# huggingface/diffusers

Measured on AMD Instinct MI355X. Metric: images/sec @ SDXL-base 1024x1024 50-step EulerDiscrete CFG bf16, higher is better.
Workload: dtype bf16; 1 GPU; SDXL-base-1.0 U-Net (2567 M params) x 50 EulerDiscrete steps, CFG 5.0 (batch 2), 128x128 latents + AutoencoderKL decode to 1024x1024; 1 prompt per GPU; global_batch=1, parallelism=dp1 (independent prompts, replicas), denoise_steps=50, output_type=pt, hip_graph=True, output_finite=True, rccl_ranks=1, tuned_live=0, cpu_binding=none

## Files before the change

### diffusers_amd/csrc/gemm.hip

```cpp
#include "gemm_kernel.cuh"
#include "gemm2_shared.cuh"

namespace da_gemm {
int dispatch_conv(const da_gemm_params& p, int tile, int staging, hipStream_t s);
}
namespace da_gemm2 {
int dispatch_lin(const da_gemm_params& p, int tile, int staging, hipStream_t s);
int dispatch_conv(const da_gemm_params& p, int tile, int staging, hipStream_t s);
}
namespace da_gemm3 {
int dispatch_lin(const da_gemm_params& p, int tile, int staging, hipStream_t s);
}

namespace {

struct TileShape {
  int bm, bn, waves;
};
constexpr TileShape kTiles[] = {{0, 0, 0},      {128, 128, 4}, {64, 128, 4},  {128, 64, 4}, {64, 64, 4},
                                {256, 128, 8},  {128, 256, 8}, {256, 256, 8}, {128, 128, 8},
                                {128, 128, 8},  {128, 80, 8},  {128, 160, 8}, {80, 128, 8}, {128, 64, 8},
                                {128, 320, 8},  {256, 128, 8}, {128, 256, 8}, {256, 160, 8}, {256, 256, 8}, {256, 320, 8},
                                {256, 256, 8},  {256, 320, 8}};
static_assert(sizeof(kTiles) / sizeof(kTiles[0]) == DA_TILE_COUNT, "kTiles / DA_TILE_* mismatch");
inline bool is_k3(int tile) { return tile == DA_TILE_K3_256x256 || tile == DA_TILE_K3_256x320; }
inline bool is_k2(int tile) { return tile >= DA_TILE_K2_128x128 && !is_k3(tile); }
constexpr int kNumTiles = sizeof(kTiles) / sizeof(kTiles[0]);

int pick_tile(const da_gemm_params& p) {
  auto nblk = [&](int t) {
    return (long)((p.M + kTiles[t].bm - 1) / kTiles[t].bm) * ((p.N + kTiles[t].bn - 1) / kTiles[t].bn);
  };
  const bool geglu = (p.act == DA_ACT_GEGLU || p.act == DA_ACT_GEGLU_TANH);
  const bool narrow = !geglu && ((p.N & 127) != 0) && ((p.N % 128) <= 64);
  if (narrow) return (nblk(DA_TILE_128x64) >= 200) ? DA_TILE_128x64 : DA_TILE_64x64;
  if (nblk(DA_TILE_256x128) >= 480) return DA_TILE_256x128;
  if (nblk(DA_TILE_128x128) >= 128) return DA_TILE_128x128;
  if (nblk(DA_TILE_64x128) >= 128 || geglu) return DA_TILE_64x128;
  return DA_TILE_64x64;
}

int validate_conv(const da_gemm_params& p) {
  if (p.C1 <= 0 || (p.C1 & 63) || (p.C2 & 63) || p.C2 < 0) return DA_ERR_UNSUPPORTED;
  if (p.conv != 1 && p.conv != 3) return DA_ERR_UNSUPPORTED;
  if (p.K != p.conv * p.conv * (p.C1 + p.C2)) return DA_ERR_INVALID;
  if (p.stride != 1 && p.stride != 2) return DA_ERR_UNSUPPORTED;
  if (p.up != 0 && p.up != 1) return DA_ERR_INVALID;
  if (p.Hin <= 0 || p.Win <= 0 || p.Hout <= 0 || p.Wout <= 0) return DA_ERR_INVALID;
  if (p.M % (p.Hout * p.Wout)) return DA_ERR_INVALID;
  return DA_OK;
}

int validate(da_gemm_params& p) {
  if (p.M <= 0 || p.N <= 0 || p.K <= 0) return DA_ERR_INVALID;
  if ((p.K & 63) || (p.N & 3) || (p.ldc & 3)) return DA_ERR_UNSUPPORTED;
  if (!p.A || !p.W || !p.C) return DA_ERR_INVALID;
  if (p.residual && (p.ldr & 3)) return DA_ERR_UNSUPPORTED;
  if (p.rowvec && (p.rows_per_batch <= 0 || (p.ld_rowvec & 3))) return DA_ERR_INVALID;
  if (p.gate && (p.rows_per_batch <= 0 || (p.ld_gate & 3))) return DA_ERR_INVALID;
  if (p.alpha == 0.0f) p.alpha = 1.0f;
  if (p.out_scale == 0.0f) p.out_scale = 1.0f;
  if (p.conv) {
    const int v = validate_conv(p);
    if (v != DA_OK) return v;
    if (p.C2 > 0 && !p.A2) return DA_ERR_INVALID;
  } else {
    if ((p.lda & 7) || (p.ldw & 7)) return DA_ERR_UNSUPPORTED;
  }
  if ((p.act == DA_ACT_GEGLU || p.act == DA_ACT_GEGLU_TANH) &&
      ((p.N & 127) || p.out_f32 || p.residual || p.rowvec || p.gate || p.bias_rows))
    return DA_ERR_UNSUPPORTED;
  if (p.act < 0 || p.act > DA_ACT_GEGLU_TANH) return DA_ERR_INVALID;
  if (p.split_k < 0 || p.split_k > DA_SPLITK_MAX) return DA_ERR_INVALID;
  if (p.split_k > 1 && (p.stats_out || p.ln_stats)) return DA_ERR_UNSUPPORTED;
  if (p.k_valid < 0 || (p.k_valid > 0 && (p.k_valid > (p.conv ? p.C1 : p.K) || (p.conv && p.C2 != 0)))) return DA_ERR_INVALID;
  if (p.stats_out && (p.conv || p.out_f32 || p.act == DA_ACT_GEGLU || p.act == DA_ACT_GEGLU_TANH || p.stats_ld <= 0 || (p.stats_ld & 1)))
    return DA_ERR_UNSUPPORTED;
  if (p.ln_stats && (p.conv || !p.ln_s || !p.ln_c || p.ln_parts <= 0 || p.ln_parts > 4 * DA_LN_PAIR_LOADS ||
                     p.ln_stats_ld < 2 * DA_LN_MAX_PARTS || (p.ln_stats_ld & 3)))
    return DA_ERR_INVALID;
  return DA_OK;
}

int stats_parts(const da_gemm_params& p, int tile) {
  if (is_k2(tile)) {
    const int band = (tile == DA_TILE_K2_128x80 || tile == DA_TILE_K2_128x160) ? 80 : 0;
    return band ? (p.N + band - 1) / band : 0;
  }
  return (p.N + kTiles[tile].bn - 1) / kTiles[tile].bn;
}

bool tile_ok(const da_gemm_params& p, int tile) {
  if (tile <= 0 || tile >= kNumTiles) return false;
  if (is_k3(tile)) {
    if (p.conv || p.split_k > 1 || p.stats_out || (p.ln_stats && tile != DA_TILE_K3_256x320) || p.vt || p.xa_k) return false;
    if (tile == DA_TILE_K3_256x320)
      return (p.act == DA_ACT_GEGLU || p.act == DA_ACT_GEGLU_TANH) && (p.M % 256) == 0 && (p.N % 320) == 0 && !(p.ldc & 7) &&
             !((size_t)p.C & 15);
    return true;
  }
  if (is_k2(tile)) {
    const bool geglu = (p.act == DA_ACT_GEGLU || p.act == DA_ACT_GEGLU_TANH);
    const bool geglu_ok = tile == DA_TILE_K2_128x128 || tile == DA_TILE_K1_256x128 || tile == DA_TILE_K1_128x256 ||
                          tile == DA_TILE_K1_256x256 || tile == DA_TILE_K1_256x320 || (tile == DA_TILE_K1_128x320 && !p.conv);
    const bool lnf_lin = tile == DA_TILE_K2_128x80 || tile == DA_TILE_K2_128x160;
    const bool lnf_cons = lnf_lin || tile == DA_TILE_K1_128x256 || tile == DA_TILE_K1_256x128;
    if (p.xa_k) return !p.conv && p.split_k <= 1 && !geglu && !p.stats_out && !p.vt && tile == DA_TILE_K2_128x128;
    if (p.vt) return !p.conv && p.split_k <= 1 && !geglu && !p.stats_out && lnf_cons;
    if (p.stats_out || p.ln_stats) {
      if (p.conv || p.split_k > 1) return false;
      if (p.stats_out && (geglu || !lnf_lin)) return false;
      return geglu ? tile == DA_TILE_K1_128x320 : lnf_cons;
    }
    return p.split_k <= 1 && (!geglu || geglu_ok) &&
           !(p.conv && (tile == DA_TILE_K2_80x128 || tile == DA_TILE_K1_256x256 || tile == DA_TILE_K1_256x320));
  }
  if (p.vt || p.xa_k) return false;
  if ((p.act == DA_ACT_GEGLU || p.act == DA_ACT_GEGLU_TANH) &&
      (tile == DA_TILE_128x64 || tile == DA_TILE_64x64 || tile == DA_TILE_128x128_W8))
    return false;
  if (tile == DA_TILE_256x256 && (p.stats_out || p.ln_stats)) return false;
  return true;
}

__global__ __launch_bounds__(256) void touch_kernel(const uint4* __restrict__ src, size_t n, unsigned* __restrict__ sink) {
  unsigned acc = 0;
  for (size_t i = (size_t)blockIdx.x * 256 + threadIdx.x; i < n; i += (size_t)gridDim.x * 256) {
    const uint4 v = src[i];
    acc ^= v.x ^ v.y ^ v.z ^ v.w;
  }
  if (acc == 0x9e3779b9u) sink[0] = acc;
}

int run(const da_gemm_params& p, int tile, int staging, hipStream_t s, const da_gemm_params* pb = nullptr) {
  if (is_k3(tile)) return pb ? DA_ERR_UNSUPPORTED : da_gemm3::dispatch_lin(p, tile, staging, s);
  if (is_k2(tile)) {
    if (pb) return DA_ERR_UNSUPPORTED;
    return p.conv ? da_gemm2::dispatch_conv(p, tile, staging, s) : da_gemm2::dispatch_lin(p, tile, staging, s);
  }
  if (p.conv) return pb ? DA_ERR_UNSUPPORTED : da_gemm::dispatch_conv(p, tile, staging, s);
  return da_gemm::dispatch<false>(p, tile, staging, s, pb);
}

}

extern "C" int da_gemm_bf16(const da_gemm_params* pp, void* stream) {
  if (!pp) return DA_ERR_INVALID;
  da_gemm_params p = *pp;
  const int v = validate(p);
  if (v != DA_OK) return v;
  int tile = p.tile;
  if (tile == DA_TILE_AUTO) tile = pick_tile(p);
  if (!tile_ok(p, tile)) return DA_ERR_UNSUPPORTED;
  if (p.stats_out && (stats_parts(p, tile) <= 0 || p.stats_ld < 2 * stats_parts(p, tile))) return DA_ERR_INVALID;
  return run(p, tile, p.staging, (hipStream_t)stream);
}

extern "C" int da_gemm_stats_parts(const da_gemm_params* pp) {
  if (!pp || pp->N <= 0) return 0;
  int tile = pp->tile;
  if (tile == DA_TILE_AUTO) tile = pick_tile(*pp);
  if (tile <= 0 || tile >= kNumTiles) return 0;
  return stats_parts(*pp, tile);
}

extern "C" int da_conv_chunk_channels(const da_gemm_params* pp, int tile) {
  if (!pp || !pp->conv || pp->M <= 0 || pp->N <= 0) return -DA_ERR_INVALID;
  const da_gemm_params& p = *pp;
  const int v = validate_conv(p);
  if (v != DA_OK) return -v;
  if (!is_k2(tile) || !tile_ok(p, tile)) return -DA_ERR_UNSUPPORTED;
  return da_gemm2::conv_chunk_channels(p, kTiles[tile].bm, kTiles[tile].bn);
}

extern "C" int da_gemm_pair_bf16(const da_gemm_params* pa, const da_gemm_params* pb, void* stream) {
  if (!pa || !pb) return DA_ERR_INVALID;
  da_gemm_params a = *pa, b = *pb;
  int v = validate(a);
  if (v != DA_OK) return v;
  v = validate(b);
  if (v != DA_OK) return v;
  if (a.conv || b.conv || a.split_k > 1 || b.split_k > 1) return DA_ERR_UNSUPPORTED;
  int tile = a.tile;
  if (tile == DA_TILE_AUTO) tile = pick_tile(a);
  if (!tile_ok(a, tile) || !tile_ok(b, tile)) return DA_ERR_UNSUPPORTED;
  return run(a, tile, a.staging, (hipStream_t)stream, &b);
}

extern "C" int da_gemm_tune(const da_gemm_params* pp, const da_gemm_params* pair, void* stream, int iters, void* scratch,
                            size_t scratch_bytes, int* best_tile, int* best_staging, int* best_split, float* best_us) {
  if (!pp || !best_tile || !best_staging) return DA_ERR_INVALID;
  da_gemm_params p = *pp;
  int v = validate(p);
  if (v != DA_OK) return v;
  da_gemm_params pb{};
  if (pair) {
    pb = *pair;
    v = validate(pb);
    if (v != DA_OK) return v;
    if (p.conv || pb.conv) return DA_ERR_UNSUPPORTED;
  }
  if (iters <= 0) iters = 3;
  hipStream_t s = (hipStream_t)stream;
  hipEvent_t e0, e1;
  if (hipEventCreate(&e0) != hipSuccess || hipEventCreate(&e1) != hipSuccess) return DA_ERR_LAUNCH;
  float best = 3.0e38f;
  int bt = 0, bs = 0, bk = 1;
  static const int stagings[] = {DA_STAGE_LDS_DIRECT, DA_STAGE_LDS_DIRECT3, DA_STAGE_LDS_DIRECT4, DA_STAGE_LDS_DIRECT6,
                                 DA_STAGE_LDS_DIRECT8, DA_STAGE_PINGPONG, DA_STAGE_PINGPONG3};
  constexpr int n_stagings = sizeof(stagings) / sizeof(stagings[0]);
  static const int splits[] = {1, 2, 3, 4, 6, 8, 12, 16, 24};
  const int n_splits = (best_split && !pair && p.workspace && p.sync_flags) ? (int)(sizeof(splits) / sizeof(splits[0])) : 1;
  const int family = pp->tile;
  for (int spi = 0; spi < n_splits; ++spi) {
    const int split = splits[spi];
    p.split_k = split;
    for (int tile = 1; tile < kNumTiles; ++tile) {
      if ((family == DA_TILE_FAMILY_1 && (is_k2(tile) || is_k3(tile))) || (family == DA_TILE_FAMILY_K2 && !is_k2(tile) && !is_k3(tile))) continue;
      if (!tile_ok(p, tile) || (pair && !tile_ok(pb, tile))) continue;
      if (kTiles[tile].bm >= 2 * p.M + 64 || kTiles[tile].bn >= 2 * p.N + 64) continue;
      if (split > 1) {
        const long tiles = (long)((p.M + kTiles[tile].bm - 1) / kTiles[tile].bm) * ((p.N + kTiles[tile].bn - 1) / kTiles[tile].bn);
        if (tiles >= 256 || (p.K >> 6) < 4 * split) continue;
      }
      for (int si = 0; si < n_stagings; ++si) {
        const int st = stagings[si];
        int rc = run(p, tile, st, s, pair ? &pb : nullptr);
        if (rc == DA_ERR_UNSUPPORTED || (split > 1 && rc == DA_ERR_INVALID)) continue;
        if (rc != DA_OK) { (void)hipEventDestroy(e0); (void)hipEventDestroy(e1); return rc; }
        float tmin = 3.0e38f;
        for (int it = 0; it < iters; ++it) {
          if (scratch && scratch_bytes) {
            (void)hipMemsetAsync(scratch, 0, scratch_bytes, s);
            const da_gemm_params* both[2] = {&p, pair ? &pb : nullptr};
            for (int w = 0; w < 2; ++w) {
              if (!both[w]) continue;
              const da_gemm_params& q = *both[w];
              const size_t na = q.conv ? (size_t)(q.M / ((size_t)q.Hout * q.Wout)) * q.Hin * q.Win * q.C1 * 2
                                       : ((size_t)(q.M - 1) * q.lda + q.K) * 2;
              if (na <= ((size_t)192 << 20))
                DA_LAUNCH(touch_kernel, dim3(1024), dim3(256), 0, s, (const uint4*)q.A, na / 16, (unsigned*)scratch);
            }
          }
          (void)hipEventRecord(e0, s);
          rc = run(p, tile, st, s, pair ? &pb : nullptr);
          (void)hipEventRecord(e1, s);
          if (rc != DA_OK || hipEventSynchronize(e1) != hipSuccess) { (void)hipEventDestroy(e0); (void)hipEventDestroy(e1); return DA_ERR_LAUNCH; }
          float ms = 0.f;
          (void)hipEventElapsedTime(&ms, e0, e1);
          if (ms < tmin) tmin = ms;
        }
        const float score = split > 1 ? tmin * 1.03f : tmin;
        if (score < best) { best = score; bt = tile; bs = st; bk = split; }
      }
    }
  }
  (void)hipEventDestroy(e0);
  (void)hipEventDestroy(e1);
  if (bt == 0) return DA_ERR_UNSUPPORTED;
  *best_tile = bt;
  *best_staging = bs;
  if (best_split) *best_split = bk;
  if (best_us) *best_us = best * 1000.0f;
  return DA_OK;
}
```

### diffusers_amd/csrc/gemm2_kernel.cuh

```cuda
#pragma once
#include <cstdlib>
#include <type_traits>

#include "common.cuh"
#include "diffusers_amd.h"
#include "gemm2_shared.cuh"

namespace da_gemm2 {


#if defined(DA_GEMM2_TRACE)
__device__ unsigned long long* g_da2_trace;
#define DA2_TRACE(i) tr_[i] = __builtin_readcyclecounter()
#else
#define DA2_TRACE(i) ((void)0)
#endif



template <int KG, int WM, int WN, int MT, int NT, int NSLOT, bool CONV, bool PP = false, bool STREAMW = false, bool GIL = false,
          bool LNF = false, int XA = 0>
__global__ __launch_bounds__(512) void igemm2_bf16_kernel(const da_gemm_params p, const int xcd_gx_chunk) {
#if defined(__HIP_DEVICE_COMPILE__)
  const int xcd_gx = xcd_gx_chunk & 255;
  static_assert((KG == 1 || KG == 2) && KG * WM * WN == 8, "eight waves: one or two K-groups");
  constexpr int BM = 16 * MT * WM, BN = 16 * NT * WN;
  constexpr int PX = BM / 8, PW = BN / 8;
  constexpr int XBYTES = BM * 128, SLICE = (BM + BN) * 128, PAIR = KG * SLICE;
  static_assert(!PP || KG == 2, "ping-pong is a property of the two K-groups");
  static_assert(!STREAMW || (KG == 1 && NSLOT == 2 && !CONV), "streaming-W loop: one K-group, two-slice ring, nn.Linear");
  static_assert(!GIL || (KG == 1 && !CONV && WN == 2 && (NT % 2) == 0), "GEGLU-interleaved ownership: two wave columns, value / gate tile pairs");
  static_assert(!LNF || (!CONV && !STREAMW), "LayerNorm fold: nn.Linear instantiations of the ring loops");
  static_assert(XA == 0 || (LNF && KG == 2 && WM == 2 && WN == 2 && MT == 4 && NT == 4 && NSLOT == 2 && XA <= 8),
                "cross-attention epilogue: the 128 x 128 two-K-group tile (a wave finishes 32 rows x one 64-wide head)");
  constexpr int SW = PP ? 4 : 8;
  constexpr int UX = PP ? PX : KG * PX, UW = PP ? PW : KG * PW;
  constexpr int XI = (UX + SW - 1) / SW, WI = (UW + SW - 1) / SW;
  constexpr int XRAG = UX % SW ? 1 : 0, WRAG = UW % SW ? 1 : 0;
  static_assert(NSLOT == 2 || NSLOT == 3, "ring of 2 or 3 slice pairs");
  constexpr int DUMP = 1024;
  constexpr int LNSC = LNF ? 2 * BN * 4 : 0;
  constexpr int XA_K_OFF = 4 * MT * NT * 1024, XA_KB = XA * 16 * 128, XA_V_OFF = XA_K_OFF + 32768;
  static_assert(XA == 0 || (2 * XA_KB <= 32768 && XA_V_OFF + 32768 <= NSLOT * PAIR), "cross-attention operands do not fit the ring");
  static_assert(NSLOT * PAIR + DUMP + LNSC <= 160 * 1024, "LDS ring exceeds the 160 KiB of a CU");
  static_assert(BM % 8 == 0 && BN % 8 == 0, "tile rows are staged in 8-row pieces");
  static_assert(!CONV || (UX % SW) == 0, "conv: the slice of an activation piece must be a compile-time constant");
  static_assert((NSLOT - 1) * (XI + WI) <= 63, "vmcnt is a 6-bit counter");
  static_assert(KG == 1 || MT * NT * 1024 * 4 <= NSLOT * PAIR, "partial-sum exchange does not fit the ring");
  extern __shared__ __attribute__((aligned(16))) unsigned char smem[];

#if defined(DA_GEMM2_TRACE)
  unsigned long long tr_[8] = {0, 0, 0, 0, 0, 0, 0, 0};
#endif
  DA2_TRACE(0);
  const int t = threadIdx.x;
  const int lane = t & 63, wave = __builtin_amdgcn_readfirstlane(t >> 6);
  const int g = KG == 2 ? wave >> 2 : 0, wq = KG == 2 ? wave & 3 : wave;
  const int wm = wq / WN, wn = wq - wm * WN;
  const int r16 = lane & 15, kq = lane >> 4;

  const int tiles_n = (p.N + BN - 1) / BN, tiles_m = (p.M + BM - 1) / BM;
  const int gyn = 8 / xcd_gx;
  const int tm_per = (tiles_m + gyn - 1) / gyn, tn_per = (tiles_n + xcd_gx - 1) / xcd_gx;
  const int bid = (int)blockIdx.x;
  const int xcd = bid & 7, kblk = bid >> 3;
  const int gy = xcd / xcd_gx, gx = xcd - gy * xcd_gx;
  const int lm = kblk / tn_per, ln = kblk - lm * tn_per;
  const int tm = gy * tm_per + lm, tn = gx * tn_per + ln;
  if (tm >= tiles_m || tn >= tiles_n) return;
  const int m0 = tm * BM, n0 = tn * BN;

  const uint16_t* __restrict__ A = (const uint16_t*)p.A;
  const uint16_t* __restrict__ A2 = (const uint16_t*)p.A2;
  const uint16_t* __restrict__ Wt = (const uint16_t*)p.W;
  const int nk = p.K >> 6;
  const int nk2 = (nk + KG - 1) / KG;
  const int Ctot = CONV ? (p.C1 + p.C2) : 0;
  const int Hv = CONV ? (p.Hin << p.up) : 0, Wv = CONV ? (p.Win << p.up) : 0;

  int x_h[XI], x_r[XI], w_h[WI], w_r[WI];
  bool x_ok[XI], w_ok[WI];
#pragma unroll
  for (int i = 0; i < XI; ++i) {
    const int q = i * SW + (PP ? wq : wave);
    x_ok[i] = (i * SW + SW - 1 < UX) ? true : (q < UX);
    x_h[i] = (KG == 1 || PP) ? 0 : (i * 8 >= PX) ? 1 : (i * 8 + 7 < PX) ? 0 : (q >= PX ? 1 : 0);
    x_r[i] = q - x_h[i] * PX;
    if (!x_ok[i]) x_h[i] = 0, x_r[i] = 0;
  }
#pragma unroll
  for (int i = 0; i < WI; ++i) {
    const int q = i * SW + (PP ? wq : wave);
    w_ok[i] = (i * SW + SW - 1 < UW) ? true : (q < UW);
    w_h[i] = (KG == 1 || PP) ? 0 : (i * 8 >= PW) ? 1 : (i * 8 + 7 < PW) ? 0 : (q >= PW ? 1 : 0);
    w_r[i] = q - w_h[i] * PW;
    if (!w_ok[i]) w_h[i] = 0, w_r[i] = 0;
  }
  const int own_half = PP ? g * SLICE : 0;
  constexpr int my_loads = XI + WI;

  int xr_base[XI], xr_oy[XI], xr_ox[XI];
  if constexpr (CONV) {
    const int hw = p.Hout * p.Wout;
#pragma unroll
    for (int i = 0; i < XI; ++i) {
      const int m = m0 + x_r[i] * 8 + (lane >> 3);
      if (m < p.M) {
        const int b = m / hw;
        const int rem = m - b * hw;
        const int oy = rem / p.Wout;
        xr_base[i] = b * p.Hin;
        xr_oy[i] = oy * p.stride - p.pad;
        xr_ox[i] = (rem - oy * p.Wout) * p.stride - p.pad;
      } else {
        xr_base[i] = 0;
        xr_oy[i] = -100000;
        xr_ox[i] = -100000;
      }
    }
  }

  size_t xbase = 0, xbytes = 0x7fffffff, x2bytes = 0x7fffffff;
  int pb = 0;
  if constexpr (CONV) {
    const int hw = p.Hout * p.Wout;
    const int b0 = m0 / hw;
    const int oy0 = (m0 - b0 * hw) / p.Wout;
    pb = __builtin_amdgcn_readfirstlane((b0 * p.Hin + (max(0, oy0 * p.stride - p.pad) >> p.up)) * p.Win);
    const size_t pix_left = (size_t)(p.M / hw) * p.Hin * p.Win - (size_t)pb;
    xbytes = min(pix_left * p.C1 * 2, (size_t)0x7fffffff);
    x2bytes = min(pix_left * p.C2 * 2, (size_t)0x7fffffff);
  } else {
    xbase = (size_t)m0 * p.lda;
  }
  __amdgpu_buffer_rsrc_t rs_x = uniform_rsrc(A + (CONV ? (size_t)pb * p.C1 : xbase), xbytes);
  __amdgpu_buffer_rsrc_t rs_x2 = uniform_rsrc((CONV && A2) ? A2 + (size_t)pb * p.C2 : A, x2bytes);
  __amdgpu_buffer_rsrc_t rs_w = uniform_rsrc(Wt + (size_t)n0 * p.ldw, 0x7fffffff);

  int vo_x[XI], vo_x2[XI], vo_w[WI];
#pragma unroll
  for (int i = 0; i < XI; ++i) {
    const int row = x_r[i] * 8 + (lane >> 3);
    const int sc = (lane & 7) ^ ((row >> 1) & 7);
    if constexpr (!CONV) vo_x[i] = (min(row, p.M - 1 - m0) * p.lda + sc * 8) * 2;
    else vo_x[i] = 0;
    vo_x2[i] = 0;
  }
#pragma unroll
  for (int i = 0; i < WI; ++i) {
    const int row = w_r[i] * 8 + (lane >> 3);
    const int sc = (lane & 7) ^ ((row >> 1) & 7);
    vo_w[i] = (min(row, p.N - 1 - n0) * p.ldw + sc * 8) * 2;
  }
  const int cchunk = CONV ? (((xcd_gx_chunk >> 8) > 0 && p.conv > 1) ? min((xcd_gx_chunk >> 8) * 64, Ctot) : Ctot) : 0;
  int c_kh[2] = {0, 0}, c_kw[2] = {0, 0}, c_c0[2] = {0, 0};
  int c_beg[2] = {0, 0}, c_end[2] = {cchunk, cchunk};
  int st_pr = 0;
  int st_s[2] = {PP ? min(g, nk - 1) : 0, nk > 1 ? 1 : 0};
  int st_zero[2] = {(!PP || g < nk) ? 0 : (int)0x80000000, (nk > 1) ? 0 : (int)0x80000000};
  auto tap_offsets = [&](int h) {
#pragma unroll
    for (int i = 0; i < XI; ++i) {
      if ((KG == 2 && !PP && i >= XI / 2 ? 1 : 0) != h) continue;
      const int row = x_r[i] * 8 + (lane >> 3);
      const int sc = (lane & 7) ^ ((row >> 1) & 7);
      const int iy = xr_oy[i] + c_kh[h], ix = xr_ox[i] + c_kw[h];
      const bool ok = (unsigned)iy < (unsigned)Hv && (unsigned)ix < (unsigned)Wv;
      const int rel = (xr_base[i] + (iy >> p.up)) * p.Win + (ix >> p.up) - pb;
      vo_x[i] = ok ? (rel * p.C1 + sc * 8) * 2 : (int)0x80000000;
      vo_x2[i] = ok ? (rel * p.C2 + sc * 8) * 2 : (int)0x80000000;
    }
  };
  auto cursor_step = [&](int h) {
    c_c0[h] += 64;
    if (c_c0[h] >= c_end[h]) {
      if (++c_kw[h] >= p.conv) {
        c_kw[h] = 0;
        if (++c_kh[h] >= p.conv && c_end[h] < Ctot) {
          c_kh[h] = 0;
          c_beg[h] = c_end[h];
          c_end[h] = min(c_end[h] + cchunk, Ctot);
        }
      }
      c_c0[h] = c_beg[h];
    }
  };
  auto w_off = [&](int h) { return ((c_kh[h] * p.conv + c_kw[h]) * Ctot + c_c0[h]) * 2; };
  if constexpr (CONV) {
    if (PP) {
      if (g == 1 && nk > 1) cursor_step(0);
    } else if (KG == 2 && nk > 1) {
      cursor_step(1);
    }
    tap_offsets(0);
    if (KG == 2 && !PP) tap_offsets(1);
  }
  int st_woff[2] = {CONV ? w_off(0) : 0, CONV ? w_off(1) : 0};

#define DA2_LDS(ptr) ((__attribute__((address_space(3))) void*)(ptr))
  auto stage_issue_base = [&](unsigned char* base, auto which_c) {
    constexpr int WHICH = decltype(which_c)::value;
    auto issue_x = [&](auto ic) {
      constexpr int i = decltype(ic)::value;
      const int h = x_h[i];
      const int z = x_ok[i] ? (h ? st_zero[1] : st_zero[0]) : (int)0x80000000;
      unsigned char* dst = x_ok[i] ? base + own_half + h * SLICE + x_r[i] * 1024 : smem + NSLOT * PAIR;
      if constexpr (CONV) {
        const int c0 = h ? c_c0[1] : c_c0[0];
        if (p.C2 > 0 && c0 >= p.C1)
          __builtin_amdgcn_raw_ptr_buffer_load_lds(rs_x2, DA2_LDS(dst), 16, vo_x2[i] | z, (c0 - p.C1) * 2, 0, 0);
        else
          __builtin_amdgcn_raw_ptr_buffer_load_lds(rs_x, DA2_LDS(dst), 16, vo_x[i] | z, c0 * 2, 0, 0);
      } else {
        __builtin_amdgcn_raw_ptr_buffer_load_lds(rs_x, DA2_LDS(dst), 16, vo_x[i] | z, (h ? st_s[1] : st_s[0]) * 128, 0, 0);
      }
    };
    auto issue_w = [&](auto ic) {
      constexpr int i = decltype(ic)::value;
      const int h = w_h[i];
      const int z = w_ok[i] ? (h ? st_zero[1] : st_zero[0]) : (int)0x80000000;
      unsigned char* dst = w_ok[i] ? base + own_half + h * SLICE + XBYTES + w_r[i] * 1024 : smem + NSLOT * PAIR;
      if constexpr (CONV)
        __builtin_amdgcn_raw_ptr_buffer_load_lds(rs_w, DA2_LDS(dst), 16, vo_w[i] | z, h ? st_woff[1] : st_woff[0], 0, 0);
      else
        __builtin_amdgcn_raw_ptr_buffer_load_lds(rs_w, DA2_LDS(dst), 16, vo_w[i] | z, (h ? st_s[1] : st_s[0]) * 128, 0, 0);
    };
    if constexpr (WHICH >= 0) {
      if constexpr (WHICH < WI) issue_w(std::integral_constant<int, WHICH < WI ? WHICH : 0>{});
      else issue_x(std::integral_constant<int, WHICH >= WI ? WHICH - WI : 0>{});
    } else {
      static_for<XI>(issue_x);
      static_for<WI>(issue_w);
    }
  };
  auto stage_issue = [&](int slot) { stage_issue_base(smem + slot * PAIR, std::integral_constant<int, -1>{}); };
  auto stage_issue_one = [&](unsigned char* base, auto k_c) { stage_issue_base(base, k_c); };
  auto stage_advance = [&]() {
    ++st_pr;
#pragma unroll
    for (int h = 0; h < (PP ? 1 : KG); ++h) {
      const int want = min(KG * st_pr + (PP ? g : h), nk - 1);
      if constexpr (CONV) {
        const int kh0 = c_kh[h], kw0 = c_kw[h];
        while (st_s[h] < want) {
          cursor_step(h);
          ++st_s[h];
        }
        if (c_kh[h] != kh0 || c_kw[h] != kw0) tap_offsets(h);
        st_woff[h] = w_off(h);
      } else {
        st_s[h] = want;
      }
    }
    st_zero[0] = (KG * st_pr + (PP ? g : 0) < nk) ? 0 : (int)0x80000000;
    st_zero[1] = (KG * st_pr + 1 < nk) ? 0 : (int)0x80000000;
  };
#define DA2_WAIT_PAIRS(PAIRS) asm volatile("s_waitcnt vmcnt(%0)" ::"n"((PAIRS) * my_loads) : "memory")

  constexpr bool SPLIT_M = KG == 1 || (MT % 2) == 0;
  static_assert(SPLIT_M || (NT % 2) == 0, "one of the wave tile's dimensions must split between the two K-groups");
  constexpr int MH = (KG == 2 && SPLIT_M) ? MT / 2 : MT, NH = (KG == 1 || SPLIT_M) ? NT : NT / 2;
  const bool geglu = (p.act == DA_ACT_GEGLU || p.act == DA_ACT_GEGLU_TANH);
  auto row_of = [&](int ih) { return m0 + (wm * MT + (SPLIT_M ? g * MH : 0) + ih) * 16 + r16; };
  auto col_tile = [&](int jh) { return GIL ? 4 * (jh >> 1) + 2 * (jh & 1) + wn : wn * NT + (SPLIT_M ? 0 : g * NH) + jh; };
  auto col_of = [&](int jh) { return n0 + col_tile(jh) * 16 + 4 * kq; };
  constexpr bool PF = MH * NH <= (CONV ? 8 : 12);
  constexpr bool STG = NH >= 2;
  constexpr int PPR = 2 * NH, NPIECE = 16 * PPR, TT = (NPIECE + 63) / 64, ROWB = NH * 64 + 32;
  static_assert(!STG || (KG == 2 ? 4 * MT * NT * 1024 : 0) + 8 * 16 * ROWB <= NSLOT * PAIR, "output staging does not fit the ring");
  constexpr int STATS_OFF = (KG == 2 ? 4 * MT * NT * 1024 : 0) + 8 * 16 * ROWB;
  static_assert(!(LNF && STG) || STATS_OFF + 8 * TT * 64 * 8 <= NSLOT * PAIR, "statistics scratch does not fit the ring");
  const bool wide = STG && !GIL && !geglu && !p.out_f32 && !(p.ldc & 7) && !((size_t)p.C & 15) && !(p.N & 7) &&
                    (!p.residual || (!(p.ldr & 7) && !((size_t)p.residual & 15)));
  const int band_col0 = n0 + (wn * NT + (SPLIT_M ? 0 : g * NH)) * 16;
  auto band_row0 = [&](int ih) { return m0 + (wm * MT + (SPLIT_M ? g * MH : 0) + ih) * 16; };
  constexpr bool PFN = PF && !STG;
  uint2 res_v[PFN ? MH : 1][PFN ? NH : 1], bias_v[NH], rowvec_v[PF ? MH : 1][PF ? NH : 1];
  uint4 resw[(PF && STG) ? MH : 1][(PF && STG) ? TT : 1];
#pragma unroll
  for (int ih = 0; ih < (PF ? MH : 1); ++ih)
#pragma unroll
    for (int jh = 0; jh < (PF ? NH : 1); ++jh) rowvec_v[ih][jh] = make_uint2(0, 0);
#pragma unroll
  for (int ih = 0; ih < (PFN ? MH : 1); ++ih)
#pragma unroll
    for (int jh = 0; jh < (PFN ? NH : 1); ++jh) res_v[ih][jh] = make_uint2(DA_NEG0_BF2, DA_NEG0_BF2);
#pragma unroll
  for (int ih = 0; ih < ((PF && STG) ? MH : 1); ++ih)
#pragma unroll
    for (int t = 0; t < ((PF && STG) ? TT : 1); ++t) resw[ih][t] = make_uint4(DA_NEG0_BF2, DA_NEG0_BF2, DA_NEG0_BF2, DA_NEG0_BF2);
#pragma unroll
  for (int jh = 0; jh < NH; ++jh) bias_v[jh] = make_uint2(0, 0);
  constexpr bool LN_PF = LNF;
  float4 lnq[LN_PF ? MH : 1][3];
#pragma unroll
  for (int ih = 0; ih < (LN_PF ? MH : 1); ++ih)
#pragma unroll
    for (int u = 0; u < 3; ++u) lnq[ih][u] = make_float4(0.f, 0.f, 0.f, 0.f);
  auto ln_load = [&](int ih, float4* dst) {
    const int m = min(row_of(ih), p.M - 1);
    const float* sp = p.ln_stats + (size_t)m * p.ln_stats_ld;
#pragma unroll
    for (int u = 0; u < 3; ++u) dst[u] = *(const float4*)(sp + ((6 * kq + 2 * u < p.ln_parts) ? 12 * kq + 4 * u : 0));
  };
  float4 lnsc_v = make_float4(0.f, 0.f, 0.f, 0.f);
  auto prefetch_epilogue_operands = [&]() {
    if constexpr (LNF) {
      if (p.ln_stats) {
        if (t < BN / 2) {
          const int j = t < BN / 4 ? t : t - BN / 4;
          const int n = min(n0 + 4 * j, p.N - 4);
          lnsc_v = *(const float4*)((t < BN / 4 ? p.ln_s : p.ln_c) + n);
        }
      }
    }
    if constexpr (LN_PF) {
      if (p.ln_stats) {
#pragma unroll
        for (int ih = 0; ih < MH; ++ih) ln_load(ih, lnq[ih]);
      }
    }
    const uint16_t* __restrict__ resid = (const uint16_t*)p.residual;
    const uint16_t* __restrict__ bias = (const uint16_t*)p.bias;
    const uint16_t* __restrict__ rowvec = (const uint16_t*)p.rowvec;
    if constexpr (PFN) {
      if (resid) {
#pragma unroll
        for (int ih = 0; ih < MH; ++ih) {
          const int m = min(row_of(ih), p.M - 1);
#pragma unroll
          for (int jh = 0; jh < NH; ++jh) res_v[ih][jh] = *(const uint2*)(resid + (size_t)m * p.ldr + min(col_of(jh), p.N - 4));
        }
      }
    }
    if constexpr (PF && STG) {
      if (resid && wide) {
#pragma unroll
        for (int ih = 0; ih < MH; ++ih)
#pragma unroll
          for (int t = 0; t < TT; ++t) {
            const int q = (NPIECE % 64 == 0) ? lane + 64 * t : min(lane + 64 * t, NPIECE - 1);
            const int m = min(band_row0(ih) + q / PPR, p.M - 1), n = min(band_col0 + (q % PPR) * 8, p.N - 8);
            resw[ih][t] = *(const uint4*)(resid + (size_t)m * p.ldr + n);
          }
      }
    }
    if (!STREAMW && bias) {
#pragma unroll
      for (int jh = 0; jh < NH; ++jh) bias_v[jh] = *(const uint2*)(bias + min(col_of(jh), p.N - 4));
    }
    if (PF && rowvec) {
#pragma unroll
      for (int ih = 0; ih < (PF ? MH : 0); ++ih) {
        const int m = min(row_of(ih), p.M - 1);
        const size_t ro = (size_t)(m / p.rows_per_batch) * p.ld_rowvec;
#pragma unroll
        for (int jh = 0; jh < NH; ++jh) rowvec_v[ih][jh] = *(const uint2*)(rowvec + ro + min(col_of(jh), p.N - 4));
      }
    }
  };

  f32x4_t acc[MT][NT];
#pragma unroll
  for (int i = 0; i < MT; ++i)
#pragma unroll
    for (int j = 0; j < NT; ++j) acc[i][j] = f32x4_t{0.f, 0.f, 0.f, 0.f};

  const int fsw = (r16 >> 1) & 7;
  const int foff0 = r16 * 128 + ((kq ^ fsw) << 4), foff1 = r16 * 128 + (((kq ^ fsw) ^ 4) << 4);
  const int xfrag = g * SLICE + (wm * MT) * 2048, wfrag = g * SLICE + XBYTES + (GIL ? wn : wn * NT) * 2048;
  auto wtile_off = [](int j) { return (GIL ? 4 * (j >> 1) + 2 * (j & 1) : j) * 2048; };
  bf16x8_t xf0[MT], wf0[NT], xf1[MT], wf1[NT];
#define DA2_FRAG(XF, WF, SLOT, OFF)                                                                         \
  do {                                                                                                      \
    const unsigned char* xb_ = smem + (SLOT) * PAIR + xfrag + (OFF);                                        \
    const unsigned char* wb_ = smem + (SLOT) * PAIR + wfrag + (OFF);                                        \
    _Pragma("unroll") for (int j = 0; j < NT; ++j) WF[j] = *(const bf16x8_t*)(wb_ + wtile_off(j));          \
    _Pragma("unroll") for (int i = 0; i < MT; ++i) XF[i] = *(const bf16x8_t*)(xb_ + i * 2048);              \
  } while (0)
#define DA2_MFMA(XF, WF)                                                                                    \
  do {                                                                                                      \
    _Pragma("unroll") for (int i = 0; i < MT; ++i)                                                          \
    _Pragma("unroll") for (int j = 0; j < NT; ++j)                                                          \
      acc[i][j] = __builtin_amdgcn_mfma_f32_16x16x32_bf16(WF[j], XF[i], acc[i][j], 0, 0, 0);                \
  } while (0)
#define DA2_SG_DS(n) __builtin_amdgcn_sched_group_barrier(0x100, n, 0)
#define DA2_SG_MF(n) __builtin_amdgcn_sched_group_barrier(0x008, n, 0)
#define DA2_SG_VM(n) __builtin_amdgcn_sched_group_barrier(0x020, n, 0)

  DA2_TRACE(1);
#pragma unroll
  for (int s = 0; s < (STREAMW ? 1 : NSLOT); ++s) {
    stage_issue(s);
    stage_advance();
    if (s == 0) prefetch_epilogue_operands();
  }
  DA2_TRACE(2);
  DA2_WAIT_PAIRS(STREAMW ? 0 : NSLOT - 1);
  __builtin_amdgcn_s_barrier();
  asm volatile("" ::: "memory");
  DA2_TRACE(3);
  float ln_mu[MH], ln_rs[MH];
#pragma unroll
  for (int ih = 0; ih < MH; ++ih) ln_mu[ih] = 0.f, ln_rs[ih] = 1.f;
  const bool ln_on = LNF && p.ln_stats != nullptr;
  if constexpr (LNF) {
    if (ln_on) {
      if (t < BN / 2) {
        float* lnsc = (float*)(smem + NSLOT * PAIR + DUMP);
        const int j = t < BN / 4 ? t : t - BN / 4;
        *(float4*)(lnsc + (t < BN / 4 ? 0 : BN) + 4 * j) = lnsc_v;
      }
      const float inv_c = 1.0f / (float)p.K;
#pragma unroll
      for (int ih = 0; ih < MH; ++ih) {
        float s1 = 0.f, s2 = 0.f;
#pragma unroll
        for (int u = 0; u < 3; ++u) {
          const int q = 6 * kq + 2 * u;
          s1 += (q < p.ln_parts ? lnq[ih][u].x : 0.f) + (q + 1 < p.ln_parts ? lnq[ih][u].z : 0.f);
          s2 += (q < p.ln_parts ? lnq[ih][u].y : 0.f) + (q + 1 < p.ln_parts ? lnq[ih][u].w : 0.f);
        }
        s1 += __shfl_xor(s1, 16, 64);
        s2 += __shfl_xor(s2, 16, 64);
        s1 += __shfl_xor(s1, 32, 64);
        s2 += __shfl_xor(s2, 32, 64);
        const float mean = s1 * inv_c;
        ln_mu[ih] = mean;
        ln_rs[ih] = rsqrtf(fmaxf(s2 * inv_c - mean * mean, 0.f) + p.ln_eps);
      }
    }
  }
  if constexpr (STREAMW) {
    constexpr int QD = 2;
    constexpr int NG = 2 * NT;
    static_assert(XI + WI <= NG, "one LDS-DMA per MFMA group at most");
    const unsigned char* xbase_ = smem + xfrag, * wbase_ = smem + wfrag;
    auto wfrag_at = [&](const unsigned char* wb, int gi) {
      return *(const bf16x8_t*)(wb + wtile_off(gi % NT) + (gi < NT ? foff0 : foff1));
    };
    auto slice_body = [&](auto doff_c, int slot) __attribute__((always_inline)) {
      constexpr int DOFF = decltype(doff_c)::value;
      static_assert(DOFF + XI + WI <= NG, "LDS-DMA window past the end of the slice");
      const unsigned char* xb = xbase_ + slot * PAIR;
      const unsigned char* wb = wbase_ + slot * PAIR;
      bf16x8_t xs[2][MT], wq[QD + 1];
#pragma unroll
      for (int i = 0; i < MT; ++i) xs[0][i] = *(const bf16x8_t*)(xb + i * 2048 + foff0);
#pragma unroll
      for (int q = 0; q < QD; ++q) wq[q] = wfrag_at(wb, q);
#pragma unroll
      for (int i = 0; i < MT; ++i) xs[1][i] = *(const bf16x8_t*)(xb + i * 2048 + foff1);
      __builtin_amdgcn_sched_barrier(0);
      unsigned char* nbase = smem + (slot ^ 1) * PAIR;
      static_for<NG>([&](auto gc) {
        constexpr int gi = decltype(gc)::value, ks = gi / NT, j = gi % NT;
        if constexpr (gi + QD < NG) wq[(gi + QD) % (QD + 1)] = wfrag_at(wb, gi + QD);
        if constexpr (gi >= DOFF && gi < DOFF + XI + WI) stage_issue_one(nbase, std::integral_constant<int, gi - DOFF>{});
#pragma unroll
        for (int i = 0; i < MT; ++i)
          acc[i][j] = __builtin_amdgcn_mfma_f32_16x16x32_bf16(wq[gi % (QD + 1)], xs[ks][i], acc[i][j], 0, 0, 0);
        __builtin_amdgcn_sched_barrier(0);
      });
    };
    auto slice_loop = [&](auto doff_c) __attribute__((always_inline)) {
      int slot = 0;
      for (int sl = 0; sl < nk2; ++sl) {
        slice_body(doff_c, slot);
        __builtin_amdgcn_sched_barrier(0);
        stage_advance();
        if (sl + 1 < nk2) {
          asm volatile("s_waitcnt lgkmcnt(0)" ::: "memory");
          DA2_WAIT_PAIRS(0);
          __builtin_amdgcn_s_barrier();
          asm volatile("" ::: "memory");
        }
        slot ^= 1;
      }
    };
    if (wave < 4) slice_loop(std::integral_constant<int, 0>{});
    else slice_loop(std::integral_constant<int, NG - (XI + WI) - 3>{});
  } else {
  DA2_FRAG(xf0, wf0, 0, foff0);

  auto first_half_pins = [&]() {
    static_for<MT + NT>([](auto rc) {
      constexpr int r = decltype(rc)::value, R = MT + NT, Q = MT * NT;
      DA2_SG_DS(1);
      DA2_SG_MF((Q * (r + 1)) / R - (Q * r) / R);
    });
  };
  if constexpr (PP) {
    if (g == 1) {
      __builtin_amdgcn_s_barrier();
      asm volatile("" ::: "memory");
    }
  }
  int slot = 0;
  for (int pr = 0; pr + 1 < nk2; ++pr) {
    DA2_FRAG(xf1, wf1, slot, foff1);
    DA2_MFMA(xf0, wf0);
    first_half_pins();
    __builtin_amdgcn_sched_barrier(0);
    const int nslot = (slot + 1 == NSLOT) ? 0 : slot + 1;
    asm volatile("s_waitcnt lgkmcnt(0)" ::: "memory");
    DA2_WAIT_PAIRS(NSLOT - 2);
    __builtin_amdgcn_s_barrier();
    asm volatile("" ::: "memory");
    __builtin_amdgcn_sched_barrier(0);
    stage_issue(slot);
    DA2_FRAG(xf0, wf0, nslot, foff0);
    DA2_MFMA(xf1, wf1);
    static_for<XI + WI + MT + NT>([](auto rc) {
      constexpr int r = decltype(rc)::value, V = XI + WI, R = V + MT + NT, Q = MT * NT;
      if constexpr (r < V) DA2_SG_VM(1);
      else DA2_SG_DS(1);
      DA2_SG_MF((Q * (r + 1)) / R - (Q * r) / R);
    });
    __builtin_amdgcn_sched_barrier(0);
    if constexpr (PP) {
      __builtin_amdgcn_s_barrier();
      asm volatile("" ::: "memory");
      __builtin_amdgcn_sched_barrier(0);
    }
    stage_advance();
    slot = nslot;
  }
  DA2_FRAG(xf1, wf1, slot, foff1);
  DA2_MFMA(xf0, wf0);
  first_half_pins();
  __builtin_amdgcn_sched_barrier(0);
  DA2_MFMA(xf1, wf1);
  if constexpr (PP) {
    if (g == 0) {
      __builtin_amdgcn_sched_barrier(0);
      __builtin_amdgcn_s_barrier();
      asm volatile("" ::: "memory");
    }
  }
  }
#undef DA2_FRAG
#undef DA2_MFMA

  DA2_TRACE(4);
  f32x4_t keep[MH][NH];
  if constexpr (KG == 1) {
#pragma unroll
    for (int ih = 0; ih < MH; ++ih)
#pragma unroll
      for (int jh = 0; jh < NH; ++jh) keep[ih][jh] = acc[ih][jh];
  } else {
    asm volatile("s_waitcnt vmcnt(0) lgkmcnt(0)" ::: "memory");
    __builtin_amdgcn_s_barrier();
    asm volatile("" ::: "memory");
    if constexpr (XA > 0) {
      if (p.xa_k) {
        constexpr int KP = 2 * XA, NPK = 2 * KP, NPV = 32, NP = NPK + NPV;
        const int hb = n0 >> 6, bq = m0 / p.rows_per_batch;
        __amdgpu_buffer_rsrc_t rs_k = uniform_rsrc(p.xa_k, 0x7fffffff), rs_v = uniform_rsrc(p.xa_vt, 0x7fffffff);
#pragma unroll
        for (int i = 0; i < (NP + 7) / 8; ++i) {
          const int q = i * 8 + wave;
          if (q < NPK) {
            const int hh = q >= KP ? 1 : 0, r8 = q - hh * KP;
            const int row = r8 * 8 + (lane >> 3);
// ... 38 lines not shown
#pragma unroll
      for (int jh = 0; jh < NH; ++jh) {
        const f32x4_t o = xch[(size_t)((ih * NH + jh) + (g ? MH * NH : 0)) * 64];
#pragma unroll
        for (int e = 0; e < 4; ++e) keep[ih][jh][e] += o[e];
      }
  }

  if constexpr (STREAMW) {
    if (p.bias) {
#pragma unroll
      for (int jh = 0; jh < NH; ++jh) bias_v[jh] = *(const uint2*)((const uint16_t*)p.bias + min(col_of(jh), p.N - 4));
    }
  }
  auto weight_prefetch = [&]() {
  if (p.prefetch && (PF || !p.residual)) {
    const int nchunk = (int)min((long long)0x7fffffff >> 10, p.prefetch_bytes >> 10);
    __amdgpu_buffer_rsrc_t rs_pf = uniform_rsrc(p.prefetch, (size_t)nchunk << 10);
    const int stride = (int)gridDim.x * 8;
    int c = bid * 8 + wave;
#pragma unroll
    for (int k = 0; k < 16; ++k) {
      if (c < nchunk) __builtin_amdgcn_raw_ptr_buffer_load_lds(rs_pf, DA2_LDS(smem + NSLOT * PAIR), 16, lane * 16, c << 10, 0, 0);
      c += stride;
    }
  }
  };
  const bool xa_on = XA > 0 && p.xa_k != nullptr;
  if (!xa_on) weight_prefetch();
  DA2_TRACE(5);
  auto ln_apply4 = [&](float* o, int ih, int n) __attribute__((always_inline)) {
    if constexpr (LNF) {
      if (ln_on) {
        const float* lnsc = (const float*)(smem + NSLOT * PAIR + DUMP);
        const int j = min(n - n0, BN - 4);
        const float4 sv = *(const float4*)(lnsc + j), cv = *(const float4*)(lnsc + BN + j);
        o[0] = ln_rs[ih] * (o[0] - ln_mu[ih] * sv.x) + cv.x;
        o[1] = ln_rs[ih] * (o[1] - ln_mu[ih] * sv.y) + cv.y;
        o[2] = ln_rs[ih] * (o[2] - ln_mu[ih] * sv.z) + cv.z;
        o[3] = ln_rs[ih] * (o[3] - ln_mu[ih] * sv.w) + cv.w;
      }
    }
  };
  if constexpr (XA > 0) {
    if (xa_on) {
      bf16x8_t qf[MH][2];
#pragma unroll
      for (int ih = 0; ih < MH; ++ih)
#pragma unroll
        for (int b = 0; b < 2; ++b) {
          float o8[8];
#pragma unroll
          for (int hlf = 0; hlf < 2; ++hlf) {
            const int jh = 2 * b + hlf;
            float o[4];
#pragma unroll
            for (int e = 0; e < 4; ++e) o[e] = keep[ih][jh][e] * p.alpha;
            ln_apply4(o, ih, min(col_of(jh), p.N - 4));
            const uint2 bv = bias_v[jh];
            o8[4 * hlf + 0] = o[0] + bf_lo(bv.x); o8[4 * hlf + 1] = o[1] + bf_hi(bv.x);
            o8[4 * hlf + 2] = o[2] + bf_lo(bv.y); o8[4 * hlf + 3] = o[3] + bf_hi(bv.y);
          }
          const uint4 pk = pack8(o8);
          qf[ih][b] = __builtin_bit_cast(bf16x8_t, pk);
        }
      asm volatile("s_waitcnt vmcnt(0) lgkmcnt(0)" ::: "memory");
      __builtin_amdgcn_s_barrier();
      asm volatile("" ::: "memory");
      const unsigned char* kb = smem + XA_K_OFF + wn * XA_KB;
      const unsigned char* vb = smem + XA_V_OFF + wn * 16384;
      f32x4_t sacc[XA][MH];
#pragma unroll
      for (int kt = 0; kt < XA; ++kt) {
#pragma unroll
        for (int ih = 0; ih < MH; ++ih) sacc[kt][ih] = f32x4_t{0.f, 0.f, 0.f, 0.f};
        const int R = 16 * kt + r16, sw = (R >> 1) & 7;
#pragma unroll
        for (int b = 0; b < 2; ++b) {
          const uint2 lo = *(const uint2*)(kb + R * 128 + (((4 * b + (kq >> 1)) ^ sw) << 4) + (kq & 1) * 8);
          const uint2 hi = *(const uint2*)(kb + R * 128 + (((4 * b + 2 + (kq >> 1)) ^ sw) << 4) + (kq & 1) * 8);
          const bf16x8_t kf = __builtin_bit_cast(bf16x8_t, make_uint4(lo.x, lo.y, hi.x, hi.y));
#pragma unroll
          for (int ih = 0; ih < MH; ++ih) sacc[kt][ih] = __builtin_amdgcn_mfma_f32_16x16x32_bf16(kf, qf[ih][b], sacc[kt][ih], 0, 0, 0);
        }
      }
      constexpr int KBL = (XA + 1) / 2;
      const float sl2 = p.xa_scale * 1.4426950408889634f;
      bf16x8_t pf[MH][KBL];
      float linv[MH];
#pragma unroll
      for (int ih = 0; ih < MH; ++ih) {
        float mx = -3.0e38f;
#pragma unroll
        for (int kt = 0; kt < XA; ++kt)
#pragma unroll
          for (int e = 0; e < 4; ++e) {
            const float v = (16 * kt + 4 * kq + e < p.xa_skv) ? sacc[kt][ih][e] * sl2 : -3.0e38f;
            sacc[kt][ih][e] = v;
            mx = fmaxf(mx, v);
          }
        mx = fmaxf(mx, __shfl_xor(mx, 16, 64));
        mx = fmaxf(mx, __shfl_xor(mx, 32, 64));
        float sum = 0.f;
#pragma unroll
        for (int c = 0; c < KBL; ++c) {
          float p8[8];
#pragma unroll
          for (int hlf = 0; hlf < 2; ++hlf)
#pragma unroll
            for (int e = 0; e < 4; ++e) {
              float pv = 0.f;
              if (2 * c + hlf < XA) pv = __builtin_amdgcn_exp2f(sacc[2 * c + hlf < XA ? 2 * c + hlf : 0][ih][e] - mx);
              p8[4 * hlf + e] = pv;
              sum += pv;
            }
          pf[ih][c] = __builtin_bit_cast(bf16x8_t, pack8(p8));
        }
        sum += __shfl_xor(sum, 16, 64);
        sum += __shfl_xor(sum, 32, 64);
        linv[ih] = 1.0f / sum;
      }
#pragma unroll
      for (int dt = 0; dt < 4; ++dt) {
        f32x4_t oacc[MH];
#pragma unroll
        for (int ih = 0; ih < MH; ++ih) oacc[ih] = f32x4_t{0.f, 0.f, 0.f, 0.f};
        const int Rd = 16 * dt + r16, sw = Rd & 15;
#pragma unroll
        for (int c = 0; c < KBL; ++c) {
          const uint2 lo = *(const uint2*)(vb + Rd * 256 + (((4 * c + (kq >> 1)) ^ sw) << 4) + (kq & 1) * 8);
          const uint2 hi = *(const uint2*)(vb + Rd * 256 + (((4 * c + 2 + (kq >> 1)) ^ sw) << 4) + (kq & 1) * 8);
          const bf16x8_t vf = __builtin_bit_cast(bf16x8_t, make_uint4(lo.x, lo.y, hi.x, hi.y));
#pragma unroll
          for (int ih = 0; ih < MH; ++ih) oacc[ih] = __builtin_amdgcn_mfma_f32_16x16x32_bf16(vf, pf[ih][c], oacc[ih], 0, 0, 0);
        }
#pragma unroll
        for (int ih = 0; ih < MH; ++ih)
#pragma unroll
          for (int e = 0; e < 4; ++e) keep[ih][dt][e] = oacc[ih][e] * linv[ih];
      }
      weight_prefetch();
    }
  }
  const uint16_t* __restrict__ bias_rows = (const uint16_t*)p.bias_rows;
  const bool has_rowvec = p.rowvec != nullptr, has_res = p.residual != nullptr;
#if defined(DA_GEMM2_TRACE)
#define DA2_TRACE_END()                                                                                     \
  do {                                                                                                      \
    DA2_TRACE(6);                                                                 \
    asm volatile("s_waitcnt vmcnt(0)" ::: "memory");                                                        \
    DA2_TRACE(7);                                                                 \
    if (lane == 0) {                                                                                        \
      _Pragma("unroll") for (int i = 0; i < 8; ++i) g_da2_trace[((size_t)blockIdx.x * 8 + wave) * 8 + i] = tr_[i]; \
    }                                                                                                       \
  } while (0)
#else
#define DA2_TRACE_END() ((void)0)
#endif
  if (geglu) {
    if constexpr (GIL) {
      constexpr int OROW = BN + 16;
      static_assert(BM * OROW <= NSLOT * PAIR, "output tile does not fit the ring");
      asm volatile("s_waitcnt lgkmcnt(0)" ::: "memory");
      __builtin_amdgcn_s_barrier();
      asm volatile("" ::: "memory");
      auto body = [&](auto tanh_c) __attribute__((always_inline)) {
        constexpr bool TANH = decltype(tanh_c)::value;
#pragma unroll
        for (int ih = 0; ih < MH; ++ih) {
          unsigned char* orow = smem + ((wm * MT + ih) * 16 + r16) * OROW + (wn * 16 + 4 * kq) * 2;
#pragma unroll
          for (int u = 0; u < NT / 2; ++u) {
            const uint2 bh = bias_v[2 * u], bg = bias_v[2 * u + 1];
            float o[4], hq[4], gq[4];
#pragma unroll
            for (int e = 0; e < 4; ++e) hq[e] = keep[ih][2 * u][e] * p.alpha, gq[e] = keep[ih][2 * u + 1][e] * p.alpha;
            ln_apply4(hq, ih, min(col_of(2 * u), p.N - 4));
            ln_apply4(gq, ih, min(col_of(2 * u + 1), p.N - 4));
#pragma unroll
            for (int e = 0; e < 4; ++e) {
              float hv = hq[e], gv = gq[e];
              hv += (e == 0) ? bf_lo(bh.x) : (e == 1) ? bf_hi(bh.x) : (e == 2) ? bf_lo(bh.y) : bf_hi(bh.y);
              gv += (e == 0) ? bf_lo(bg.x) : (e == 1) ? bf_hi(bg.x) : (e == 2) ? bf_lo(bg.y) : bf_hi(bg.y);
              hv = bf2f(f2bf(hv));
              gv = bf2f(f2bf(gv));
              o[e] = hv * bf2f(f2bf(TANH ? gelu_tanh_f(gv) : gelu_erf_f(gv)));
            }
            uint2 pk;
            pk.x = pack_bf2(o[0], o[1]);
            pk.y = pack_bf2(o[2], o[3]);
            *(uint2*)(orow + u * 64) = pk;
          }
        }
      };
      if (p.act == DA_ACT_GEGLU) body(std::false_type{});
      else body(std::true_type{});
      asm volatile("s_waitcnt lgkmcnt(0)" ::: "memory");
      __builtin_amdgcn_s_barrier();
      asm volatile("" ::: "memory");
      constexpr int OPR = BN / 16, NOP = BM * OPR;
      const int no0 = n0 >> 1, Nout = p.N >> 1;
#pragma unroll
      for (int k = 0; k < (NOP + 511) / 512; ++k) {
        const int q = t + 512 * k;
        if (NOP % 512 != 0 && q >= NOP) continue;
        const int row = q / OPR, c = q % OPR;
        if (m0 + row >= p.M || no0 + c * 8 >= Nout) continue;
        *(uint4*)((uint16_t*)p.C + (size_t)(m0 + row) * p.ldc + no0 + c * 8) = *(const uint4*)(smem + row * OROW + c * 16);
      }
      DA2_TRACE_END();
      return;
    }
    if constexpr (!GIL && SPLIT_M && (NT % 4) == 0) {
      auto body = [&](auto tanh_c) __attribute__((always_inline)) {
        constexpr bool TANH = decltype(tanh_c)::value;
#pragma unroll
        for (int ih = 0; ih < MH; ++ih) {
          const int m = row_of(ih);
          if (m >= p.M) continue;
#pragma unroll
          for (int u = 0; u < NT / 4; ++u)
#pragma unroll
            for (int v = 0; v < 2; ++v) {
              const int jv = 4 * u + v, jg = jv + 2;
              const int nv = col_of(jv);
              if (nv >= p.N) continue;
              const int no = (n0 >> 1) + (wn * (NT / 4) + u) * 32 + v * 16 + 4 * kq;
              const uint2 bh = bias_v[jv], bg = bias_v[jg];
              float o[4], hq[4], gq[4];
#pragma unroll
              for (int e = 0; e < 4; ++e) hq[e] = keep[ih][jv][e] * p.alpha, gq[e] = keep[ih][jg][e] * p.alpha;
              ln_apply4(hq, ih, nv);
              ln_apply4(gq, ih, col_of(jg));
#pragma unroll
              for (int e = 0; e < 4; ++e) {
                float hv = hq[e], gv = gq[e];
                hv += (e == 0) ? bf_lo(bh.x) : (e == 1) ? bf_hi(bh.x) : (e == 2) ? bf_lo(bh.y) : bf_hi(bh.y);
                gv += (e == 0) ? bf_lo(bg.x) : (e == 1) ? bf_hi(bg.x) : (e == 2) ? bf_lo(bg.y) : bf_hi(bg.y);
                hv = bf2f(f2bf(hv));
                gv = bf2f(f2bf(gv));
                o[e] = hv * bf2f(f2bf(TANH ? gelu_tanh_f(gv) : gelu_erf_f(gv)));
              }
              uint2 pk;
              pk.x = pack_bf2(o[0], o[1]);
              pk.y = pack_bf2(o[2], o[3]);
              *(uint2*)((uint16_t*)p.C + (size_t)m * p.ldc + no) = pk;
            }
        }
      };
      if (p.act == DA_ACT_GEGLU) body(std::false_type{});
      else body(std::true_type{});
    }
    return;
  }
  auto wide_body = [&](auto act_c, auto gate_c, auto packed_c) __attribute__((always_inline)) {
    constexpr int ACT = decltype(act_c)::value, GATE = decltype(gate_c)::value;
    constexpr bool PACKED = decltype(packed_c)::value;
    if constexpr (STG) {
      if constexpr (KG == 1) {
        asm volatile("s_waitcnt lgkmcnt(0)" ::: "memory");
        __builtin_amdgcn_s_barrier();
        asm volatile("" ::: "memory");
      }
      unsigned char* stg = smem + ((KG == 2 && !xa_on) ? 4 * MT * NT * 1024 : 0) + wave * (16 * ROWB);
      unsigned char* stg_w = stg + r16 * ROWB + kq * 16;
      const uint16_t* __restrict__ resid = (const uint16_t*)p.residual;
#pragma unroll
      for (int ih = 0; ih < MH; ++ih) {
        const int mc = min(row_of(ih), p.M - 1);
        const int bidx = (GATE != 0 || (!PF && has_rowvec)) ? (mc / p.rows_per_batch) : 0;
        const float brow = bias_rows ? bf2f(bias_rows[mc]) : 0.f;
#pragma unroll
        for (int jh = 0; jh < NH; ++jh) {
          const int n = min(col_of(jh), p.N - 4);
          float o[4];
          if (XA > 0 && xa_on) {
#pragma unroll
            for (int e = 0; e < 4; ++e) o[e] = keep[ih][jh][e];
          } else {
#pragma unroll
          for (int e = 0; e < 4; ++e) o[e] = keep[ih][jh][e] * p.alpha;
          ln_apply4(o, ih, n);
          uint2 rvv = make_uint2(0, 0);
          if constexpr (PF) rvv = rowvec_v[ih][jh];
          else if (has_rowvec) rvv = *(const uint2*)((const uint16_t*)p.rowvec + (size_t)bidx * p.ld_rowvec + n);
          epilogue4<ACT, GATE, false>(p, o, n, bidx, brow, bias_v[jh], rvv, make_uint2(0, 0));
          }
          if constexpr (PACKED) {
            uint2 pk;
            pk.x = pack_bf2(o[0], o[1]);
            pk.y = pack_bf2(o[2], o[3]);
            *(uint2*)(stg + r16 * (ROWB / 2) + kq * 8 + jh * 32) = pk;
          } else {
            *(float4*)(stg_w + jh * 64) = make_float4(o[0], o[1], o[2], o[3]);
          }
        }
        float2* part = (float2*)(smem + STATS_OFF) + wave * (TT * 64);
#pragma unroll
        for (int t = 0; t < TT; ++t) {
          const int q = lane + 64 * t;
          if (NPIECE % 64 != 0 && q >= NPIECE) continue;
          const int row = q / PPR, c8 = q % PPR;
          const int mo = band_row0(ih) + row, no = band_col0 + c8 * 8;
          const bool inside = mo < p.M && no < p.N;
          uint4 pk;
          if constexpr (PACKED) {
            pk = *(const uint4*)(stg + row * (ROWB / 2) + c8 * 16);
          } else {
            const float4 lo = *(const float4*)(stg + row * ROWB + c8 * 32), hi = *(const float4*)(stg + row * ROWB + c8 * 32 + 16);
            float o[8] = {lo.x, lo.y, lo.z, lo.w, hi.x, hi.y, hi.z, hi.w};
            uint4 rw = make_uint4(DA_NEG0_BF2, DA_NEG0_BF2, DA_NEG0_BF2, DA_NEG0_BF2);
            if constexpr (PF) rw = resw[ih][t];
            else if (has_res && inside) rw = *(const uint4*)(resid + (size_t)mo * p.ldr + no);
            o[0] += bf_lo(rw.x); o[1] += bf_hi(rw.x); o[2] += bf_lo(rw.y); o[3] += bf_hi(rw.y);
            o[4] += bf_lo(rw.z); o[5] += bf_hi(rw.z); o[6] += bf_lo(rw.w); o[7] += bf_hi(rw.w);
#pragma unroll
            for (int e = 0; e < 8; ++e) o[e] *= p.out_scale;
            pk.x = pack_bf2(o[0], o[1]); pk.y = pack_bf2(o[2], o[3]); pk.z = pack_bf2(o[4], o[5]); pk.w = pack_bf2(o[6], o[7]);
          }
          if (inside) *(uint4*)((uint16_t*)p.C + (size_t)mo * p.ldc + no) = pk;
          if constexpr (LNF) {
            if (p.stats_out) {
              float r[8];
              unpack8(pk, r);
              const float s1 = ((r[0] + r[1]) + (r[2] + r[3])) + ((r[4] + r[5]) + (r[6] + r[7]));
              const float s2 = ((r[0] * r[0] + r[1] * r[1]) + (r[2] * r[2] + r[3] * r[3])) +
                               ((r[4] * r[4] + r[5] * r[5]) + (r[6] * r[6] + r[7] * r[7]));
              part[q] = inside ? make_float2(s1, s2) : make_float2(0.f, 0.f);
            }
          }
        }
        if constexpr (LNF) {
          if (p.stats_out) {
            asm volatile("s_waitcnt lgkmcnt(0)" ::: "memory");
            if (lane < 16) {
              float a = 0.f, b = 0.f;
#pragma unroll
              for (int c = 0; c < PPR; ++c) {
                const float2 v = part[lane * PPR + c];
                a += v.x;
                b += v.y;
              }
              const int mo = band_row0(ih) + lane;
              if (mo < p.M && band_col0 < p.N)
                *(float2*)(p.stats_out + (size_t)mo * p.stats_ld + 2 * (band_col0 / (16 * NH))) = make_float2(a, b);
            }
            asm volatile("s_waitcnt lgkmcnt(0)" ::: "memory");
          }
        }
      }
    }
  };
  auto narrow_body = [&](auto act_c, auto gate_c) __attribute__((always_inline)) {
    constexpr int ACT = decltype(act_c)::value, GATE = decltype(gate_c)::value;
#pragma unroll
    for (int ih = 0; ih < MH; ++ih) {
      const int m = row_of(ih);
      if (m >= p.M) continue;
      const int bidx = (GATE != 0 || (!PF && has_rowvec)) ? (m / p.rows_per_batch) : 0;
      const float brow = bias_rows ? bf2f(bias_rows[m]) : 0.f;
#pragma unroll
      for (int jh = 0; jh < NH; ++jh) {
        const int n = col_of(jh);
        if (n >= p.N) continue;
        float o[4];
#pragma unroll
        for (int e = 0; e < 4; ++e) o[e] = keep[ih][jh][e] * p.alpha;
        ln_apply4(o, ih, n);
        uint2 rvv = make_uint2(0, 0), rsv = make_uint2(DA_NEG0_BF2, DA_NEG0_BF2);
        if constexpr (PF) rvv = rowvec_v[ih][jh];
        else if (has_rowvec) rvv = *(const uint2*)((const uint16_t*)p.rowvec + (size_t)bidx * p.ld_rowvec + n);
        if constexpr (PFN) rsv = res_v[ih][jh];
        else if (has_res) rsv = *(const uint2*)((const uint16_t*)p.residual + (size_t)m * p.ldr + n);
        epilogue4<ACT, GATE, true>(p, o, n, bidx, brow, bias_v[jh], rvv, rsv);
        if (p.out_f32) {
          *(float4*)((float*)p.C + (size_t)m * p.ldc + n) = make_float4(o[0], o[1], o[2], o[3]);
        } else {
          uint2 pk;
          pk.x = pack_bf2(o[0], o[1]);
          pk.y = pack_bf2(o[2], o[3]);
          *(uint2*)((uint16_t*)p.C + (size_t)m * p.ldc + n) = pk;
        }
      }
    }
  };
  if constexpr (LNF && !GIL) {
    if (p.vt && n0 >= p.vt_col0) {
      uint16_t* __restrict__ vt = (uint16_t*)p.vt;
#pragma unroll
      for (int ih = 0; ih < MH; ++ih) {
        const int m = row_of(ih);
#pragma unroll
        for (int jh = 0; jh < NH; ++jh) {
          const int n = col_of(jh);
          if (n >= p.N) continue;
          float o[4];
#pragma unroll
          for (int e = 0; e < 4; ++e) o[e] = keep[ih][jh][e] * p.alpha;
          ln_apply4(o, ih, n);
          const uint2 bv = bias_v[jh];
          o[0] += bf_lo(bv.x); o[1] += bf_hi(bv.x); o[2] += bf_lo(bv.y); o[3] += bf_hi(bv.y);
          if (m < p.M) {
            uint16_t* dst = vt + (size_t)(n - p.vt_col0) * p.ld_vt + m;
#pragma unroll
            for (int e = 0; e < 4; ++e) dst[(size_t)e * p.ld_vt] = f2bf(o[e]);
          }
        }
      }
      DA2_TRACE_END();
      return;
    }
  }
  {
    using std::integral_constant;
    auto by_act = [&](auto&& f, auto... tail) __attribute__((always_inline)) {
      if (p.act == DA_ACT_NONE) f(integral_constant<int, DA_ACT_NONE>{}, tail...);
      else if (p.act == DA_ACT_GELU_TANH) f(integral_constant<int, DA_ACT_GELU_TANH>{}, tail...);
      else if (p.act == DA_ACT_SILU) f(integral_constant<int, DA_ACT_SILU>{}, tail...);
      else if (p.act == DA_ACT_GELU_ERF) f(integral_constant<int, DA_ACT_GELU_ERF>{}, tail...);
      else f(integral_constant<int, DA_ACT_QUICK_GELU>{}, tail...);
    };
    constexpr integral_constant<int, -1> RT{};
    constexpr integral_constant<int, 0> G0{};
    if (STG && wide) {
      const bool packed = !has_res && p.out_scale == 1.0f;
      if (p.gate && p.gate_f32) wide_body(RT, integral_constant<int, 2>{}, std::false_type{});
      else if (p.gate) wide_body(RT, integral_constant<int, 1>{}, std::false_type{});
      else if (packed) by_act(wide_body, G0, std::true_type{});
      else by_act(wide_body, G0, std::false_type{});
    } else {
      if (p.gate && p.gate_f32) narrow_body(RT, integral_constant<int, 2>{});
      else if (p.gate) narrow_body(RT, integral_constant<int, 1>{});
      else if constexpr (STG) narrow_body(RT, G0);
      else by_act(narrow_body, G0);
    }
  }
  DA2_TRACE_END();
#undef DA2_TRACE_END
#undef DA2_LDS
#undef DA2_WAIT_PAIRS
#undef DA2_SG_DS
#undef DA2_SG_MF
#undef DA2_SG_VM
#endif
}



template <int KG, int WM, int WN, int MT, int NT, int NSLOT, bool CONV, bool PP = false, bool STREAMW = false, bool GIL = false,
          bool LNF = false, int XA = 0>
int launch(const da_gemm_params& p, hipStream_t s) {
  constexpr int BM = 16 * MT * WM, BN = 16 * NT * WN;
  const LaunchGeom geom = launch_geom(p, BM, BN, CONV);
  constexpr size_t lds = (size_t)NSLOT * KG * (BM + BN) * 128 + 1024 + (LNF ? 2 * BN * 4 : 0);
  auto kern = igemm2_bf16_kernel<KG, WM, WN, MT, NT, NSLOT, CONV, PP, STREAMW, GIL, LNF, XA>;
  static bool attr_set = false;
  if (!attr_set) {
    if (hipFuncSetAttribute((const void*)kern, hipFuncAttributeMaxDynamicSharedMemorySize, (int)lds) != hipSuccess)
      return DA_ERR_LAUNCH;
    attr_set = true;
  }
  DA_LAUNCH(kern, dim3(geom.grid), dim3(512), lds, s, p, geom.gx | (CONV ? conv_chunk_slices(p, geom.rows_xcd) << 8 : 0));
  DA_CHECK_LAUNCH();
  return DA_OK;
}

inline int stats_band_cols(int tile) { return (tile == DA_TILE_K2_128x80 || tile == DA_TILE_K2_128x160) ? 80 : 0; }

inline int dispatch_lnf(const da_gemm_params& p, int tile, int staging, hipStream_t s) {
  const bool geglu = (p.act == DA_ACT_GEGLU || p.act == DA_ACT_GEGLU_TANH);
  const int ns = (staging == DA_STAGE_LDS_DIRECT || staging == DA_STAGE_PINGPONG) ? 2
                 : (staging == DA_STAGE_LDS_DIRECT3 || staging == DA_STAGE_PINGPONG3) ? 3 : 0;
  const bool pp = staging == DA_STAGE_PINGPONG || staging == DA_STAGE_PINGPONG3;
  if (ns == 0) return DA_ERR_UNSUPPORTED;
  if (p.xa_k) {
    if (tile != DA_TILE_K2_128x128 || ns != 2 || geglu || !p.xa_vt || p.vt || p.stats_out || p.residual || p.gate || p.rowvec ||
        p.bias_rows || p.out_f32 || p.act != DA_ACT_NONE || p.out_scale != 1.0f || (p.N & 127) || (p.ldc & 7) ||
        ((size_t)p.C & 15) || p.rows_per_batch <= 0 || (p.rows_per_batch & 127) || (p.M % p.rows_per_batch) || p.xa_skv <= 0 ||
        p.xa_skv > p.xa_skv_alloc || p.xa_skv_alloc > 80 || (p.xa_skv_alloc & 7) || (p.xa_k_ld & 7) || (p.xa_vt_ld & 7) ||
        p.xa_k_ld < p.N || p.xa_vt_ld < (long long)(p.M / p.rows_per_batch) * p.xa_skv_alloc ||
        ((size_t)p.xa_k & 15) || ((size_t)p.xa_vt & 15) ||
        (size_t)(p.M / p.rows_per_batch) * p.xa_skv_alloc * p.xa_k_ld * 2 >= 0x7fffffffull || (size_t)p.N * p.xa_vt_ld * 2 >= 0x7fffffffull)
      return DA_ERR_UNSUPPORTED;
    return pp ? launch<2, 2, 2, 4, 4, 2, false, true, false, false, true, 5>(p, s)
              : launch<2, 2, 2, 4, 4, 2, false, false, false, false, true, 5>(p, s);
  }
  if (p.vt) {
    const int bn = tile == DA_TILE_K2_128x80 ? 80 : tile == DA_TILE_K2_128x160 ? 160 : tile == DA_TILE_K1_128x256 ? 256
                   : tile == DA_TILE_K1_256x128 ? 128 : 0;
    if (bn == 0 || geglu || p.stats_out || p.residual || p.gate || p.rowvec || p.bias_rows || p.out_f32 || p.act != DA_ACT_NONE ||
        p.vt_col0 <= 0 || p.vt_col0 >= p.N || (p.vt_col0 % bn) || (p.vt_col0 & 15) || p.ld_vt < p.M || p.out_scale != 1.0f)
      return DA_ERR_UNSUPPORTED;
  }
  if (p.stats_out) {
    if (geglu || p.out_f32 || (p.ldc & 7) || ((size_t)p.C & 15) || (p.N & 7) || p.gate ||
        (p.residual && ((p.ldr & 7) || ((size_t)p.residual & 15))) || stats_band_cols(tile) == 0)
      return DA_ERR_UNSUPPORTED;
  }
  switch (tile) {
    case DA_TILE_K2_128x80:
      if (geglu) break;
      if (pp) return ns == 2 ? launch<2, 4, 1, 2, 5, 2, false, true, false, false, true>(p, s)
                             : launch<2, 4, 1, 2, 5, 3, false, true, false, false, true>(p, s);
      return ns == 2 ? launch<2, 4, 1, 2, 5, 2, false, false, false, false, true>(p, s)
                     : launch<2, 4, 1, 2, 5, 3, false, false, false, false, true>(p, s);
    case DA_TILE_K2_128x160:
      if (geglu || ns != 2) break;
      return pp ? launch<2, 2, 2, 4, 5, 2, false, true, false, false, true>(p, s)
                : launch<2, 2, 2, 4, 5, 2, false, false, false, false, true>(p, s);
    case DA_TILE_K1_128x320:
      if (!geglu || p.stats_out || ns != 2 || pp || (p.ldc & 7) || ((size_t)p.C & 15) || (p.N & 15)) break;
      return launch<1, 4, 2, 2, 10, 2, false, false, false, true, true>(p, s);
    case DA_TILE_K1_128x256:
      if (geglu || p.stats_out || pp) break;
      return ns == 2 ? launch<1, 2, 4, 4, 4, 2, false, false, false, false, true>(p, s)
                     : launch<1, 2, 4, 4, 4, 3, false, false, false, false, true>(p, s);
    case DA_TILE_K1_256x128:
      if (geglu || p.stats_out || pp) break;
      return ns == 2 ? launch<1, 4, 2, 4, 4, 2, false, false, false, false, true>(p, s)
                     : launch<1, 4, 2, 4, 4, 3, false, false, false, false, true>(p, s);
  }
  return DA_ERR_UNSUPPORTED;
}

template <bool CONV>
int dispatch(const da_gemm_params& p, int tile, int staging, hipStream_t s) {
  if (p.split_k > 1 || !staging_fits(p)) return DA_ERR_UNSUPPORTED;
  if (p.stats_out || p.ln_stats || p.vt || p.xa_k) {
    if constexpr (CONV) return DA_ERR_UNSUPPORTED;
    else return dispatch_lnf(p, tile, staging, s);
  }
  const bool geglu = (p.act == DA_ACT_GEGLU || p.act == DA_ACT_GEGLU_TANH);
  if (geglu && tile != DA_TILE_K2_128x128 && tile != DA_TILE_K1_256x128 && tile != DA_TILE_K1_128x256 && tile != DA_TILE_K1_256x256 &&
      tile != DA_TILE_K1_256x320 && tile != DA_TILE_K1_128x320)
    return DA_ERR_UNSUPPORTED;
  const int ns = (staging == DA_STAGE_LDS_DIRECT || staging == DA_STAGE_PINGPONG) ? 2
                 : (staging == DA_STAGE_LDS_DIRECT3 || staging == DA_STAGE_PINGPONG3) ? 3 : 0;
  if (ns == 0) return DA_ERR_UNSUPPORTED;
  if (staging == DA_STAGE_PINGPONG || staging == DA_STAGE_PINGPONG3) {
    switch (tile) {
      case DA_TILE_K2_128x128:
        if (ns == 2) return launch<2, 2, 2, 4, 4, 2, CONV, true>(p, s);
        break;
      case DA_TILE_K2_128x80:
        return ns == 2 ? launch<2, 4, 1, 2, 5, 2, CONV, true>(p, s) : launch<2, 4, 1, 2, 5, 3, CONV, true>(p, s);
      case DA_TILE_K2_128x160:
        if (ns == 2) return launch<2, 2, 2, 4, 5, 2, CONV, true>(p, s);
        break;
      case DA_TILE_K2_80x128:
        if constexpr (!CONV) return ns == 2 ? launch<2, 1, 4, 5, 2, 2, false, true>(p, s) : launch<2, 1, 4, 5, 2, 3, false, true>(p, s);
        break;
      case DA_TILE_K2_128x64:
        return ns == 2 ? launch<2, 2, 2, 4, 2, 2, CONV, true>(p, s) : launch<2, 2, 2, 4, 2, 3, CONV, true>(p, s);
    }
    return DA_ERR_UNSUPPORTED;
  }
  switch (tile) {
    case DA_TILE_K2_128x128:
      if (ns == 2) return launch<2, 2, 2, 4, 4, 2, CONV>(p, s);
      break;
    case DA_TILE_K2_128x80:
      return ns == 2 ? launch<2, 4, 1, 2, 5, 2, CONV>(p, s) : launch<2, 4, 1, 2, 5, 3, CONV>(p, s);
    case DA_TILE_K2_128x160:
      if (ns == 2) return launch<2, 2, 2, 4, 5, 2, CONV>(p, s);
      break;
    case DA_TILE_K2_80x128:
      if constexpr (!CONV) return ns == 2 ? launch<2, 1, 4, 5, 2, 2, false>(p, s) : launch<2, 1, 4, 5, 2, 3, false>(p, s);
      break;
    case DA_TILE_K2_128x64:
      return ns == 2 ? launch<2, 2, 2, 4, 2, 2, CONV>(p, s) : launch<2, 2, 2, 4, 2, 3, CONV>(p, s);
    case DA_TILE_K1_128x320:
      if (ns != 2) break;
      if (!geglu) return launch<1, 4, 2, 2, 10, 2, CONV>(p, s);
      if constexpr (!CONV) {
        if ((p.ldc & 7) || ((size_t)p.C & 15) || (p.N & 15)) break;
        return launch<1, 4, 2, 2, 10, 2, false, false, false, true>(p, s);
      }
      break;
    case DA_TILE_K1_256x128:
      return ns == 2 ? launch<1, 4, 2, 4, 4, 2, CONV>(p, s) : launch<1, 4, 2, 4, 4, 3, CONV>(p, s);
    case DA_TILE_K1_128x256:
      return ns == 2 ? launch<1, 2, 4, 4, 4, 2, CONV>(p, s) : launch<1, 2, 4, 4, 4, 3, CONV>(p, s);
    case DA_TILE_K1_256x160:
      if (ns == 2) return launch<1, 4, 2, 4, 5, 2, CONV>(p, s);
      break;
    case DA_TILE_K1_256x320:
      if constexpr (!CONV) {
        if (ns != 2) break;
        if (!geglu) return launch<1, 4, 2, 4, 10, 2, false, false, true, false>(p, s);
        if ((p.ldc & 7) || ((size_t)p.C & 15) || (p.N & 15)) break;
        return launch<1, 4, 2, 4, 10, 2, false, false, true, true>(p, s);
      }
      break;
    case DA_TILE_K1_256x256:
      if constexpr (!CONV) {
        if (ns == 2) return launch<1, 2, 4, 8, 4, 2, false>(p, s);
      }
      break;
  }
  return DA_ERR_UNSUPPORTED;
}

}
```

### diffusers_amd/csrc/gemm2_shared.cuh

```cuda
#pragma once
#include <cstdlib>
#include <type_traits>

#include "common.cuh"
#include "diffusers_amd.h"

namespace da_gemm2 {

#if defined(__HIP_DEVICE_COMPILE__)
__device__ __forceinline__ __amdgpu_buffer_rsrc_t uniform_rsrc(const void* base, size_t bytes) {
  const uint64_t v = (uint64_t)base;
  const uint32_t lo = __builtin_amdgcn_readfirstlane((uint32_t)v);
  const uint32_t hi = __builtin_amdgcn_readfirstlane((uint32_t)(v >> 32));
  const int n = __builtin_amdgcn_readfirstlane((int)(bytes > 0x7fffffffull ? 0x7fffffffull : bytes));
  return __builtin_amdgcn_make_buffer_rsrc((void*)(((uint64_t)hi << 32) | lo), 0, n, 0x00020000);
}
#endif

template <int N, class F>
__device__ __forceinline__ void static_for(F&& f) {
  if constexpr (N > 0) {
    static_for<N - 1>(f);
    f(std::integral_constant<int, N - 1>{});
  }
}

constexpr uint32_t DA_NEG0_BF2 = 0x80008000u;

template <int ACT, int GATE, bool FINISH>
__device__ __forceinline__ void epilogue4(const da_gemm_params& p, float* o, int n, int bidx, float brow, uint2 bv, uint2 rv, uint2 resv) {
  o[0] += bf_lo(bv.x); o[1] += bf_hi(bv.x); o[2] += bf_lo(bv.y); o[3] += bf_hi(bv.y);
#pragma unroll
  for (int e = 0; e < 4; ++e) o[e] += brow;
  o[0] += bf_lo(rv.x); o[1] += bf_hi(rv.x); o[2] += bf_lo(rv.y); o[3] += bf_hi(rv.y);
  const int act = ACT >= 0 ? ACT : p.act;
  if (act == DA_ACT_GELU_TANH) {
#pragma unroll
    for (int e = 0; e < 4; ++e) o[e] = gelu_tanh_f(bf2f(f2bf(o[e])));
  } else if (act == DA_ACT_SILU) {
#pragma unroll
    for (int e = 0; e < 4; ++e) o[e] = silu_f(bf2f(f2bf(o[e])));
  } else if (act == DA_ACT_GELU_ERF) {
#pragma unroll
    for (int e = 0; e < 4; ++e) o[e] = gelu_erf_f(bf2f(f2bf(o[e])));
  } else if (act == DA_ACT_QUICK_GELU) {
#pragma unroll
    for (int e = 0; e < 4; ++e) {
      const float xv = bf2f(f2bf(o[e]));
      const float tv = bf2f(f2bf(1.702f * xv));
      o[e] = xv * bf2f(f2bf(1.0f / (1.0f + __expf(-tv))));
    }
  }
  if constexpr (GATE == 2) {
    const float4 gv = *(const float4*)((const float*)p.gate + (size_t)bidx * p.ld_gate + n);
    o[0] = bf2f(f2bf(o[0])) * gv.x; o[1] = bf2f(f2bf(o[1])) * gv.y;
    o[2] = bf2f(f2bf(o[2])) * gv.z; o[3] = bf2f(f2bf(o[3])) * gv.w;
  } else if constexpr (GATE == 1) {
    const uint2 gv = *(const uint2*)((const uint16_t*)p.gate + (size_t)bidx * p.ld_gate + n);
    o[0] = bf2f(f2bf(bf2f(f2bf(o[0])) * bf_lo(gv.x)));
    o[1] = bf2f(f2bf(bf2f(f2bf(o[1])) * bf_hi(gv.x)));
    o[2] = bf2f(f2bf(bf2f(f2bf(o[2])) * bf_lo(gv.y)));
    o[3] = bf2f(f2bf(bf2f(f2bf(o[3])) * bf_hi(gv.y)));
  }
  if constexpr (FINISH) {
    o[0] += bf_lo(resv.x); o[1] += bf_hi(resv.x); o[2] += bf_lo(resv.y); o[3] += bf_hi(resv.y);
#pragma unroll
    for (int e = 0; e < 4; ++e) o[e] *= p.out_scale;
  }
}

inline int choose_xcd_gx2(int tiles_m, int tiles_n, int BM, int BN, int wrow = 1, long long arow_bytes = 0) {
  static const int forced = [] { const char* v = getenv("DA_XCD_GX"); return v ? atoi(v) : 0; }();
  if (forced == 1 || forced == 2 || forced == 4 || forced == 8) return forced;
  int best = 1;
  double best_cost = 1e300;
  for (int gx = 1; gx <= 8; gx *= 2) {
    const int gy = 8 / gx;
    const int tm_per = (tiles_m + gy - 1) / gy, tn_per = (tiles_n + gx - 1) / gx;
    const double inflation = (double)(8 * tm_per * tn_per) / ((double)tiles_m * tiles_n);
    double cost = ((double)tm_per * BM + (double)tn_per * BN * wrow) * inflation * inflation;
    if (wrow > 1 && (double)tm_per * BM * (double)arow_bytes > 2.75 * 1048576.0) cost = ((double)tm_per * BM + (double)tn_per * BN) * wrow * inflation * inflation;
    if (cost < best_cost) {
      best_cost = cost;
      best = gx;
    }
  }
  return best;
}

inline int conv_chunk_slices(const da_gemm_params& p, long long rows_xcd = 0) {
  const char* v = getenv("DA_CONV_CHUNK");
  const int forced = v ? (v[0] == 'a' ? -1 : atoi(v)) : -1;
  if (p.conv <= 1) return 0;
  if (forced < 0) {
    const long long ctot = p.C1 + p.C2;
    if (rows_xcd <= 0 || rows_xcd * ctot * 2 <= 3ll * 1048576) return 0;
    const long long ch = (2ll * 1048576 / (rows_xcd * 2)) / 64;
    return (ch < 4 || ch * 64 >= ctot) ? 0 : (int)ch;
  }
  return forced > 0 ? forced / 64 : 0;
}
inline int xcd_conv_weighting(const da_gemm_params& p) {
  static const int on = [] { const char* v = getenv("DA_XCD_CONV"); return v ? atoi(v) : 1; }();
  return (on && p.conv > 1) ? p.conv * p.conv : 1;
}

struct LaunchGeom {
  int gx, grid;
  long long rows_xcd;
};
inline LaunchGeom launch_geom(const da_gemm_params& p, int BM, int BN, bool conv) {
  const int tiles_m = (p.M + BM - 1) / BM, tiles_n = (p.N + BN - 1) / BN;
  const int gx = choose_xcd_gx2(tiles_m, tiles_n, BM, BN, conv ? xcd_conv_weighting(p) : 1, conv ? (long long)(p.C1 + p.C2) * 2 : 0), gy = 8 / gx;
  const int tm_per = (tiles_m + gy - 1) / gy, tn_per = (tiles_n + gx - 1) / gx;
  const long long rows_xcd = (long long)BM * (tm_per < (32 + tn_per - 1) / tn_per ? tm_per : (32 + tn_per - 1) / tn_per);
  return {gx, 8 * tm_per * tn_per, rows_xcd};
}

inline int conv_chunk_channels(const da_gemm_params& p, int BM, int BN) {
  const int ch = 64 * conv_chunk_slices(p, launch_geom(p, BM, BN, true).rows_xcd);
  return (p.conv > 1 && ch < p.C1 + p.C2) ? ch : 0;
}

inline bool staging_fits(const da_gemm_params& p) {
  const size_t lim = 0x3fffffffull;
  if ((size_t)p.ldw * 512 >= lim || (size_t)p.K * 2 >= lim) return false;
  if (!p.conv) return (size_t)p.lda * 512 < lim;
  const size_t cmax = (size_t)(p.C1 > p.C2 ? p.C1 : p.C2);
  const size_t span = (size_t)256 * p.stride * p.stride + (size_t)(6 + 2 * p.stride) * p.Win + 64;
  return span * cmax * 2 < lim && (size_t)p.M / ((size_t)p.Hout * p.Wout) * p.Hin * p.Win < 0x7fffffffull;
}

}
```

### diffusers_amd/layers.py

```python
from __future__ import annotations

import os
from typing import Dict, Optional

import torch

from . import _lib as L
from . import ops

bf16 = torch.bfloat16


class Weights:

    def __init__(self, state_dict: Dict[str, torch.Tensor], device):
        self.sd = state_dict
        self.device = torch.device(device)
        self.used = set()

    def has(self, name: str) -> bool:
        return name in self.sd

    def get(self, name: str) -> torch.Tensor:
        if name not in self.sd:
            raise KeyError(f"missing weight '{name}' in state_dict")
        self.used.add(name)
        return self.sd[name].detach().to(device=self.device, dtype=bf16).contiguous()

    def get_f32(self, name: str) -> torch.Tensor:
        if name not in self.sd:
            raise KeyError(f"missing weight '{name}' in state_dict")
        self.used.add(name)
        return self.sd[name].detach().to(device=self.device, dtype=torch.float32).contiguous()

    def opt(self, name: str) -> Optional[torch.Tensor]:
        return self.get(name) if name in self.sd else None

    def unused(self):
        return sorted(set(self.sd.keys()) - self.used)


class Linear:

    def __init__(self, w: Weights, prefix: str):
        self.weight = w.get(prefix + ".weight")
        self.bias = w.opt(prefix + ".bias")

    def __call__(self, x, **kw):
        return ops.linear(x, self.weight, self.bias, **kw)

    @property
    def in_features(self) -> int:
        return self.weight.shape[1]

    @property
    def out_features(self) -> int:
        return self.weight.shape[0]


class Conv3x3:

    def __init__(self, w: Weights, prefix: str):
        self.weight = ops.pack_conv_weight(w.get(prefix + ".weight"))
        self.bias = w.opt(prefix + ".bias")
        self.ksize = 3

    def __call__(self, x, **kw):
        return ops.conv2d_nhwc(x, self.weight, self.bias, ksize=3, **kw)


class Conv1x1:

    def __init__(self, w: Weights, prefix: str):
        wt = w.get(prefix + ".weight")
        self.weight = wt.reshape(wt.shape[0], -1).contiguous()
        self.bias = w.opt(prefix + ".bias")

    def __call__(self, x, x2=None, **kw):
        if x2 is None:
            B, H, W_, C = x.shape
            y = ops.linear(x.view(B * H * W_, C), self.weight, self.bias, **kw)
            return y.view(B, H, W_, -1)
        return ops.conv2d_nhwc(x, self.weight, self.bias, ksize=1, x2=x2, **kw)


class GroupNorm:
    def __init__(self, w: Weights, prefix: str, groups: int, eps: float):
        self.weight = w.get(prefix + ".weight")
        self.bias = w.get(prefix + ".bias")
        self.groups, self.eps = groups, eps

    def __call__(self, x, silu=False, x2=None):
        return ops.group_norm_nhwc(x, self.weight, self.bias, self.groups, self.eps, silu=silu, x2=x2)


class LayerNorm:
    def __init__(self, w: Weights, prefix: str, eps: float = 1e-5, affine: bool = True):
        self.weight = w.get(prefix + ".weight") if affine else None
        self.bias = w.get(prefix + ".bias") if affine else None
        self.eps = eps

    def __call__(self, x, **kw):
        return ops.layer_norm(x, self.weight, self.bias, self.eps, **kw)


class ResnetBlock2D:

    def __init__(self, w: Weights, prefix: str, groups: int, eps: float, output_scale_factor: float = 1.0):
        self.norm1 = GroupNorm(w, prefix + ".norm1", groups, eps)
        self.conv1 = Conv3x3(w, prefix + ".conv1")
        self.has_temb = w.has(prefix + ".time_emb_proj.weight")
        if self.has_temb:
            self.time_emb_proj = Linear(w, prefix + ".time_emb_proj")
        self.norm2 = GroupNorm(w, prefix + ".norm2", groups, eps)
        self.conv2 = Conv3x3(w, prefix + ".conv2")
        self.shortcut = Conv1x1(w, prefix + ".conv_shortcut") if w.has(prefix + ".conv_shortcut.weight") else None
        self.out_scale = 1.0 / output_scale_factor

    def __call__(self, x, temb=None, skip=None):
        h = self.norm1(x, silu=True, x2=skip)
        tvec = None
        if self.has_temb and temb is not None:
            if isinstance(temb, ProjectedTemb):
                tvec = temb.all[:, self.temb_off:self.temb_off + self.temb_c]
            elif self.time_emb_proj is None:
                raise ValueError("ResnetBlock2D: this block's time_emb_proj lives in the model's TimeProjections; pass its output")
            else:
                tvec = ops.linear_small_m(temb, self.time_emb_proj.weight, self.time_emb_proj.bias, act_in=L.ACT_SILU)
        h = self.conv1(h, rowvec=tvec)
        h = self.norm2(h, silu=True)
        if self.shortcut is not None:
            res = self.shortcut(x, x2=skip)
        else:
            if skip is not None:
                raise ValueError("ResnetBlock2D: concat input requires a conv_shortcut")
            res = x
        return self.conv2(h, residual=res, out_scale=self.out_scale)


class ProjectedTemb:

    def __init__(self, t: torch.Tensor):
        self.all = t


class TimeProjections:

    def __init__(self, resnets):
        rs = [r for r in resnets if r.has_temb]
        self.weight = self.bias = None
        if not rs or os.environ.get("DIFFUSERS_AMD_TEMB_STACK", "1") == "0":
            return
        biased = [r.time_emb_proj.bias is not None for r in rs]
        if any(biased) and not all(biased):
            return
        self.weight = torch.cat([r.time_emb_proj.weight for r in rs], dim=0).contiguous()
        self.bias = torch.cat([r.time_emb_proj.bias for r in rs], dim=0).contiguous() if all(biased) else None
        off = 0
        for r in rs:
            r.temb_off, r.temb_c = off, r.time_emb_proj.weight.shape[0]
            off += r.temb_c
            r.time_emb_proj = None

    def __call__(self, temb: torch.Tensor):
        if self.weight is None:
            return temb
        return ProjectedTemb(ops.linear_small_m(temb, self.weight, self.bias, act_in=L.ACT_SILU))


class Downsample2D:

    def __init__(self, w: Weights, prefix: str, padding: int = 1):
        if padding not in (0, 1):
            raise ValueError("Downsample2D: padding must be 0 or 1")
        self.conv = Conv3x3(w, prefix + ".conv")
        self.padding = padding

    def __call__(self, x):
        if self.padding == 1:
            return self.conv(x, stride=2)
        return self.conv(x, stride=2, pad=0, pad_after=1)


class Upsample2D:

    def __init__(self, w: Weights, prefix: str):
        self.conv = Conv3x3(w, prefix + ".conv")

    def __call__(self, x):
        return self.conv(x, up=True)


class CrossKV:

    __slots__ = ("k", "vt", "skv", "skv_alloc", "batch", "bias", "buf")

    def __init__(self, k, vt, skv, skv_alloc, batch, bias=None, buf=None):
        self.k, self.vt, self.skv, self.skv_alloc, self.batch = k, vt, skv, skv_alloc, batch
        self.buf = buf
        self.bias = bias


KERNEL_HEAD_DIMS = (64, 96, 128, 160)


def kernel_head_dim(d: int) -> int:
    for k in KERNEL_HEAD_DIMS:
        if d <= k:
            return k
    raise ValueError(f"attention head_dim {d} exceeds the largest flash-kernel head size {KERNEL_HEAD_DIMS[-1]}")


def pad_head_rows(w: torch.Tensor, heads: int, d: int, dp: int) -> torch.Tensor:
    if d == dp:
        return w
    out = torch.zeros((heads, dp) + tuple(w.shape[1:]), device=w.device, dtype=w.dtype)
    out[:, :d] = w.view((heads, d) + tuple(w.shape[1:]))
    return out.view((heads * dp,) + tuple(w.shape[1:])).contiguous()


def pad_head_cols(w: torch.Tensor, heads: int, d: int, dp: int) -> torch.Tensor:
    if d == dp:
        return w
    out = torch.zeros((w.shape[0], heads, dp), device=w.device, dtype=w.dtype)
    out[:, :, :d] = w.view(w.shape[0], heads, d)
    return out.view(w.shape[0], heads * dp).contiguous()


class Attention:

    def __init__(self, w: Weights, prefix: str, heads: int, cross: bool):
        self.heads = heads
        self.cross = cross
        wq = w.get(prefix + ".to_q.weight")
        wk = w.get(prefix + ".to_k.weight")
        wv = w.get(prefix + ".to_v.weight")
        inner = wq.shape[0]
        self.head_dim = inner // heads
        self.kdim = kernel_head_dim(self.head_dim)
        self.inner = heads * self.kdim
        d, dp = self.head_dim, self.kdim
        wq, wk, wv = (pad_head_rows(t, heads, d, dp) for t in (wq, wk, wv))
        if cross:
            self.wq, self.wk, self.wv = wq, wk, wv
        else:
            self.wqk = torch.cat([wq, wk], dim=0).contiguous()
            self.wv = wv
            self.wqkv_ln = self.fold1 = None
        self.to_out = Linear(w, prefix + ".to_out.0")
        self.to_out.weight = pad_head_cols(self.to_out.weight, heads, d, dp)
        self.scale = self.head_dim ** -0.5

    def precompute_kv(self, ehs_pad: torch.Tensor, batch: int, skv: int, skv_alloc: int, bias=None) -> CrossKV:
        if bias is not None and self.kdim != 64:
            raise ValueError(f"encoder_attention_mask: the masked attention kernel exists for head sizes <= 64 "
                             f"(this layer: {self.head_dim})")
        rows, inner = ehs_pad.shape[0], self.wk.shape[0]
        buf = torch.empty(2 * rows * inner, device=ehs_pad.device, dtype=ehs_pad.dtype)
        k = ops.linear(ehs_pad, self.wk, out=buf[: rows * inner].view(rows, inner))
        vt = ops.linear(self.wv, ehs_pad, out=buf[rows * inner:].view(inner, rows))
        return CrossKV(k, vt, skv, skv_alloc, batch, bias, buf)

    def fold_norm(self, norm: "LayerNorm") -> None:
        self.wq_ln, self.fold = ops.fold_layernorm(self.wq, norm.weight, norm.bias, norm.eps)

    def fold_norm1(self, norm: "LayerNorm") -> None:
        if (2 * self.inner) % 80 != 0:
            return
        wqkv = torch.cat([self.wqk, self.wv], dim=0).contiguous()
        self.wqkv_ln, self.fold1 = ops.fold_layernorm(wqkv, norm.weight, norm.bias, norm.eps)

    def __call__(self, x, batch: int, seq: int, residual, kv: Optional[CrossKV] = None, stats=None, stats_out=None):
        Hh, D = self.heads, self.kdim
        if self.cross and ops.XATTN and kv.bias is None and ops.xattn_eligible(x.shape[0], self.inner, seq, D, kv.skv_alloc) \
                and kv.k.shape[1] == self.inner:
            xa = {"k": kv.k, "vt": kv.vt, "skv": kv.skv, "skv_alloc": kv.skv_alloc, "seq": seq, "scale": self.scale}
            o = ops.linear(x, self.wq_ln, ln=(stats, self.fold), xattn=xa) if stats is not None else ops.linear(x, self.wq, xattn=xa)
        elif self.cross:
            pfk = {"prefetch": kv.buf} if (getattr(ops, "KV_PREFETCH", False) and kv.buf is not None) else {}
            q = ops.linear(x, self.wq_ln, ln=(stats, self.fold), **pfk) if stats is not None else ops.linear(x, self.wq, **pfk)
            o = ops.attention(q, kv.k, kv.vt, B=batch, H=Hh, D=D, Sq=seq, Skv=kv.skv, Skv_alloc=kv.skv_alloc,
                              q_row_stride=self.inner, k_row_stride=self.inner,
                              q_batch_stride=seq * self.inner, k_batch_stride=kv.skv_alloc * self.inner,
                              vt_ld=batch * kv.skv_alloc, vt_batch_stride=kv.skv_alloc, scale=self.scale, bias=kv.bias)
        else:
            if stats is not None:
                qk, vt = ops.linear_qkv(x, self.wqkv_ln, 2 * self.inner, ln=(stats, self.fold1))
            else:
                qk, vt = ops.linear_pair({"x": x, "w": self.wqk}, {"x": self.wv, "w": x})
            o = ops.attention(qk, qk[:, self.inner:], vt, B=batch, H=Hh, D=D, Sq=seq, Skv=seq, Skv_alloc=seq,
                              q_row_stride=2 * self.inner, k_row_stride=2 * self.inner,
                              q_batch_stride=seq * 2 * self.inner, k_batch_stride=seq * 2 * self.inner,
                              vt_ld=batch * seq, vt_batch_stride=seq, scale=self.scale)
        return self.to_out(o, residual=residual, stats_out=stats_out)


class FeedForwardGEGLU:

    def __init__(self, w: Weights, prefix: str, norm: Optional["LayerNorm"] = None):
        w1, b1 = w.get(prefix + ".net.0.proj.weight"), w.opt(prefix + ".net.0.proj.bias")
        wp, bp = ops.pack_geglu(w1, b1)
        self.w1, self.b1 = wp, bp
        self.out = Linear(w, prefix + ".net.2")
        self.w1_ln = self.fold = None
        if norm is not None:
            wl, fold = ops.fold_layernorm(w1, norm.weight, norm.bias, norm.eps)
            wl, _ = ops.pack_geglu(wl, None)
            n = w1.shape[0] // 2
            idx = torch.arange(n, device=w1.device).view(n // 32, 32)
            order = torch.cat([idx, idx + n], dim=1).reshape(-1)
            self.w1_ln = wl
            self.fold = ops.LNFold(fold.s.index_select(0, order).contiguous(), fold.c.index_select(0, order).contiguous(),
                                   fold.eps)

    def folds_here(self, rows: int) -> bool:
        if self.w1_ln is None:
            return False
        return int(ops.LN_FOLD) == 1 or ops.geglu_fold_on_k3(rows, self.w1_ln.shape[0], self.w1_ln.shape[1])

    def __call__(self, x, residual, stats=None, stats_out=None):
        if stats is not None:
            h = ops.linear(x, self.w1_ln, self.b1, act=L.ACT_GEGLU, ln=(stats, self.fold))
        else:
            h = ops.linear(x, self.w1, self.b1, act=L.ACT_GEGLU)
        return self.out(h, residual=residual, stats_out=stats_out)


class BasicTransformerBlock:

    def __init__(self, w: Weights, prefix: str, heads: int):
        self.norm1 = LayerNorm(w, prefix + ".norm1")
        self.attn1 = Attention(w, prefix + ".attn1", heads, cross=False)
        self.norm2 = LayerNorm(w, prefix + ".norm2")
        self.attn2 = Attention(w, prefix + ".attn2", heads, cross=True)
        self.norm3 = LayerNorm(w, prefix + ".norm3")
        self.folded = int(ops.LN_FOLD)
        self.ff = FeedForwardGEGLU(w, prefix + ".ff", norm=self.norm3 if self.folded in (1, 3) else None)
        if self.folded:
            self.attn2.fold_norm(self.norm2)
            self.attn1.fold_norm1(self.norm1)
        self.folds_norm1 = bool(self.folded) and self.attn1.wqkv_ln is not None

    def __call__(self, x, batch, seq, kv: CrossKV, stats_in=None, stats_out=None):
        mode = int(ops.LN_FOLD)
        if mode and (not self.folded or (mode in (1, 3) and self.folded not in (1, 3))):
            raise RuntimeError("ops.LN_FOLD was switched on after this model was loaded: the folded weights are built at "
                               "load_state_dict() time (set DIFFUSERS_AMD_LN_FOLD / ops.LN_FOLD before loading)")
        if not mode:
            x = self.attn1(self.norm1(x), batch, seq, residual=x)
            x = self.attn2(self.norm2(x), batch, seq, residual=x, kv=kv)
            return self.ff(self.norm3(x), residual=x)
        use1 = stats_in is not None and self.folds_norm1
        if mode == 2:
            st1 = ops.RowStats(x.shape[0], x.device)
            if use1:
                x = self.attn1(x, batch, seq, residual=x, stats=stats_in, stats_out=st1)
            else:
                x = self.attn1(self.norm1(x), batch, seq, residual=x, stats_out=st1)
            x = self.attn2(x, batch, seq, residual=x, kv=kv, stats=st1)
            return self.ff(self.norm3(x), residual=x, stats_out=stats_out)
        fold3 = self.ff.folds_here(x.shape[0])
        st1 = ops.RowStats(x.shape[0], x.device)
        st2 = ops.RowStats(x.shape[0], x.device) if fold3 else None
        if use1:
            x = self.attn1(x, batch, seq, residual=x, stats=stats_in, stats_out=st1)
        else:
            x = self.attn1(self.norm1(x), batch, seq, residual=x, stats_out=st1)
        x = self.attn2(x, batch, seq, residual=x, kv=kv, stats=st1, stats_out=st2)
        if fold3:
            return self.ff(x, residual=x, stats=st2, stats_out=stats_out)
        return self.ff(self.norm3(x), residual=x, stats_out=stats_out)


class Transformer2DModel:

    def __init__(self, w: Weights, prefix: str, heads: int, layers: int, groups: int):
        self.norm = GroupNorm(w, prefix + ".norm", groups, 1e-6)
        pw = w.get(prefix + ".proj_in.weight")
        self.proj_in_w = pw.reshape(pw.shape[0], -1).contiguous()
        self.proj_in_b = w.opt(prefix + ".proj_in.bias")
        self.blocks = [BasicTransformerBlock(w, f"{prefix}.transformer_blocks.{i}", heads) for i in range(layers)]
        pw = w.get(prefix + ".proj_out.weight")
        self.proj_out_w = pw.reshape(pw.shape[0], -1).contiguous()
        self.proj_out_b = w.opt(prefix + ".proj_out.bias")

    def precompute_kv(self, ehs_pad, batch, skv, skv_alloc, bias=None):
        return [blk.attn2.precompute_kv(ehs_pad, batch, skv, skv_alloc, bias) for blk in self.blocks]

    def __call__(self, x, kvs):
        B, H, W_, C = x.shape
        res = x.view(B * H * W_, C)
        h = self.norm(x).view(B * H * W_, C)
        chain = bool(ops.LN_FOLD) and ops.LN_FOLD_NORM1 and all(b.folds_norm1 for b in self.blocks)
        st = ops.RowStats(h.shape[0], h.device) if chain else None
        h = ops.linear(h, self.proj_in_w, self.proj_in_b, stats_out=st)
        for i, (blk, kv) in enumerate(zip(self.blocks, kvs)):
            nxt = ops.RowStats(h.shape[0], h.device) if chain and i + 1 < len(self.blocks) else None
            h = blk(h, B, H * W_, kv, stats_in=st, stats_out=nxt)
            st = nxt
        h = ops.linear(h, self.proj_out_w, self.proj_out_b, residual=res)
        return h.view(B, H, W_, C)


class TimestepEmbedding:

    def __init__(self, w: Weights, prefix: str):
        self.l1 = Linear(w, prefix + ".linear_1")
        self.l2 = Linear(w, prefix + ".linear_2")

    def __call__(self, x, residual=None):
        h = ops.linear_small_m(x, self.l1.weight, self.l1.bias, act_out=L.ACT_SILU)
        return ops.linear_small_m(h, self.l2.weight, self.l2.bias, residual=residual)

    @property
    def linear_1(self) -> Linear:
        return self.l1

    @property
    def linear_2(self) -> Linear:
        return self.l2


def encoder_mask_bias(mask: torch.Tensor, batch: int, skv: int) -> torch.Tensor:
    if mask.dim() == 2:
        bias = (1 - mask.to(bf16)) * -10000.0
    elif mask.dim() == 3 and mask.shape[1] == 1:
        bias = mask[:, 0].to(bf16)
    else:
        raise ValueError("encoder_attention_mask must be [batch][key_tokens] or a [batch][1][key_tokens] bias")
    if bias.shape[0] != batch or bias.shape[1] != skv:
        raise ValueError(f"encoder_attention_mask shape {tuple(mask.shape)} does not match ({batch}, {skv}) text tokens")
    out = torch.zeros((batch, 1, 1, (skv + 63) // 64 * 64), device=mask.device, dtype=bf16)
    out[:, 0, 0, :skv] = bias
    return out


def pad_encoder_states(ehs: torch.Tensor):
    B, S, C = ehs.shape
    s_alloc = ((S + 15) // 16) * 16
    if s_alloc == S:
        return ehs.reshape(B * S, C).contiguous(), S, s_alloc
    pad = torch.zeros((B, s_alloc, C), device=ehs.device, dtype=ehs.dtype)
    pad[:, :S].copy_(ehs)
    return pad.view(B * s_alloc, C), S, s_alloc
```

### diffusers_amd/loading.py

```python
from __future__ import annotations

import hashlib
import json
import os
import warnings
from collections.abc import Mapping
from pathlib import Path
from typing import Dict, Iterator, List, Optional

import torch

from . import packed_cache

CONFIG_NAME = "config.json"
WEIGHTS_NAME = "diffusion_pytorch_model"
PACKED_DIR = "diffusers_amd_packed"


class LazyCheckpoint(Mapping):

    def __init__(self, files: List[Path], device: str = "cpu"):
        from safetensors import safe_open
        self._files = [Path(f) for f in files]
        self._device = device
        self._where: Dict[str, Path] = {}
        for f in self._files:
            with safe_open(str(f), framework="pt") as h:
                for k in h.keys():
                    if k in self._where:
                        raise ValueError(f"tensor {k!r} appears in both {self._where[k].name} and {f.name}")
                    self._where[k] = f

    def __getitem__(self, key: str) -> torch.Tensor:
        from safetensors import safe_open
        f = self._where[key]
        with safe_open(str(f), framework="pt", device=self._device) as h:
            return h.get_tensor(key)

    def __iter__(self) -> Iterator[str]:
        return iter(self._where)

    def __len__(self) -> int:
        return len(self._where)

    def __contains__(self, key) -> bool:
        return key in self._where


COMPONENT_PREFIXES = ("unet.", "transformer.", "text_encoder.", "text_encoder_2.", "text_encoder_3.")
_LORA_TAGS = ((".lora_A.weight", ".lora_B.weight"), (".lora_A.default.weight", ".lora_B.default.weight"),
              (".lora.down.weight", ".lora.up.weight"), ("_lora.down.weight", "_lora.up.weight"),
              (".lora_down.weight", ".lora_up.weight"))


def _lora_pairs(lora_sd: Mapping, prefixes=("unet.", "transformer."), strict: bool = False) -> Dict[str, dict]:
    out: Dict[str, dict] = {}
    keys = list(lora_sd)
    prefixed = any(k.startswith(COMPONENT_PREFIXES) for k in keys)

    def strip(k: str):
        if not prefixed:
            return k
        for p in prefixes:
            if k.startswith(p):
                return k[len(p):]
        return None

    for k in keys:
        name = strip(k)
        if name is None:
            continue
        base = which = None
        for a_tag, b_tag in _LORA_TAGS:
            if name.endswith(a_tag):
                base, which, legacy = name[: -len(a_tag)], "A", a_tag.startswith("_lora")
            elif name.endswith(b_tag):
                base, which, legacy = name[: -len(b_tag)], "B", b_tag.startswith("_lora")
            else:
                continue
            break
        if base is None:
            if name.endswith(".alpha"):
                out.setdefault(name[: -len(".alpha")], {})["alpha"] = float(torch.as_tensor(lora_sd[k]).item())
            continue
        if legacy:
            base = base.replace(".processor.", ".")
            if base.endswith(".to_out"):
                base += ".0"
        out.setdefault(base, {})[which] = lora_sd[k]
    bad = [m for m, v in out.items() if "A" not in v or "B" not in v]
    if bad:
        raise ValueError(f"LoRA state dict has unpaired matrices for {bad[:4]}")
    if prefixed and not out:
        msg = (f"No LoRA keys found under {prefixes}; the file's components are "
               f"{sorted({k.split('.', 1)[0] for k in keys})}")
        if strict:
            raise ValueError(msg)
        warnings.warn(msg + " -- this model is left unchanged", stacklevel=2)
    return out


class LoraFusedView(Mapping):

    def __init__(self, base: Mapping, lora_sd: Mapping, scale: float = 1.0):
        self.base, self.scale = base, float(scale)
        self.pairs = _lora_pairs(lora_sd)
        unknown = [m for m in self.pairs if m + ".weight" not in base]
        if unknown:
            raise KeyError(f"LoRA targets modules the checkpoint does not have: {unknown[:4]} (of {len(unknown)})")

    def __getitem__(self, key: str) -> torch.Tensor:
        w = self.base[key]
        if not key.endswith(".weight"):
            return w
        ent = self.pairs.get(key[: -len(".weight")])
        if ent is None:
            return w
        a, b = ent["A"].to(torch.float32), ent["B"].to(torch.float32)
        r = a.shape[0]
        s = self.scale * ((ent["alpha"] / r) if ent.get("alpha") is not None else 1.0)
        if w.dim() == 4:
            delta = (b.reshape(b.shape[0], r) @ a.reshape(r, -1)).reshape(w.shape)
        else:
            delta = b @ a
        if tuple(delta.shape) != tuple(w.shape):
            raise ValueError(f"LoRA delta {tuple(delta.shape)} does not fit {key} {tuple(w.shape)}")
        return (w.to(torch.float32) + s * delta.to(w.device)).to(w.dtype)

    def __iter__(self):
        return iter(self.base)

    def __len__(self):
        return len(self.base)

    def __contains__(self, key):
        return key in self.base


def _resolve_dir(name_or_path, subfolder: Optional[str]) -> Path:
    p = Path(name_or_path)
    if not p.exists():
        try:
            from huggingface_hub import snapshot_download
            p = Path(snapshot_download(str(name_or_path), allow_patterns=["*.json", "*.safetensors"]))
        except Exception as e:
            raise OSError(f"{name_or_path!r} is not a local directory and could not be fetched from the Hub: {e}") from e
    if subfolder:
        p = p / subfolder
    if not (p / CONFIG_NAME).exists():
        raise OSError(f"{p} has no {CONFIG_NAME}")
    return p


def _weight_files(d: Path, variant: Optional[str], stem: str = WEIGHTS_NAME) -> List[Path]:
    base = stem
    stem = base + (f".{variant}" if variant else "")
    single = d / f"{stem}.safetensors"
    if single.exists():
        return [single]
    index = d / f"{stem}.safetensors.index.json"
    if not index.exists():
        index = d / f"{base}.safetensors.index{'.' + variant if variant else ''}.json"
    if index.exists():
        files = sorted(set(json.loads(index.read_text())["weight_map"].values()))
        return [d / f for f in files]
    if (d / f"{stem}.bin").exists():
        raise OSError(f"{d} holds a pickle checkpoint ({stem}.bin); convert it to safetensors (the engine does not unpickle)")
    raise OSError(f"no {stem}.safetensors (or sharded index) in {d}")


def checkpoint_fingerprint(files: List[Path], extra: str = "") -> str:
    h = hashlib.sha256(extra.encode())
    for f in sorted(files):
        st = f.stat()
        h.update(f.name.encode())
        h.update(str((st.st_size, st.st_mtime_ns)).encode())
        with open(f, "rb") as fh:
            n = int.from_bytes(fh.read(8), "little")
            h.update(fh.read(min(n, 1 << 20)))
            step = max(4096, (st.st_size // 64) & ~4095)
            for off in range(0, st.st_size, step):
                fh.seek(off)
                h.update(fh.read(4096))
    return h.hexdigest()[:24]


def read_config(d: Path) -> dict:
    cfg = json.loads((d / CONFIG_NAME).read_text())
    return {k: (tuple(v) if isinstance(v, list) else v) for k, v in cfg.items() if not k.startswith("_")}


class PretrainedMixin:

    _source: Optional[dict] = None

    @classmethod
    def from_pretrained(cls, pretrained_model_name_or_path, subfolder: Optional[str] = None, torch_dtype=None,
                        variant: Optional[str] = None, device="cuda", use_safetensors: Optional[bool] = None,
                        cache_packed: bool = True, cache_dir: Optional[os.PathLike] = None, **config_overrides):
        if torch_dtype not in (None, torch.bfloat16):
            raise ValueError(f"{cls.__name__}.from_pretrained: torch_dtype={torch_dtype} -- the HIP engine computes in bfloat16")
        if use_safetensors is False:
            raise ValueError(f"{cls.__name__}.from_pretrained: pickle checkpoints are not read; use safetensors")
        from .config_utils import from_reference_config
        d = _resolve_dir(pretrained_model_name_or_path, subfolder)
        files = _weight_files(d, variant)
        cfg = read_config(d)
        cfg.update(config_overrides)
        from . import ops
        fp = checkpoint_fingerprint(files, extra=cls.__name__ + json.dumps(cfg, sort_keys=True, default=str)
                                    + (f"+lnfold{int(ops.LN_FOLD)}qkv" if ops.LN_FOLD else "") + "+tembcat")
        cdir = Path(cache_dir) if cache_dir is not None else d / PACKED_DIR
        cfile = cdir / f"{cls.__name__}-{fp}.safetensors"
        model = None
        if cache_packed and cfile.exists():
            try:
                model = packed_cache.load_packed(cls, cfile, device=device, expect_fingerprint=fp)
            except ValueError:
                model = None
        if model is None:
            model = from_reference_config(cls, cfg)
            model.load_state_dict(LazyCheckpoint(files), device=device)
            if cache_packed:
                try:
                    packed_cache.save_packed(model, cfile, source_fingerprint=fp)
                except OSError:
                    pass
        model._source = {"files": [str(f) for f in files]}
        model._lora = None
        return model

    def _base_view(self) -> Mapping:
        if not self._source:
            raise RuntimeError(f"{type(self).__name__}: built from an in-memory state_dict; pass `base_state_dict=` "
                               "(the reference-format weights are not kept after packing)")
        return LazyCheckpoint([Path(f) for f in self._source["files"]])

    def _repack_in_place(self, view: Mapping) -> None:
        fresh = type(self)(**{k: v for k, v in dict(self.config).items()})
        fresh.load_state_dict(view, device="cpu")
        old, new = packed_cache.packed_tensors(self), packed_cache.packed_tensors(fresh)
        if list(old) != list(new):
            raise RuntimeError("re-pack produced a different tensor inventory")
        for k, t in old.items():
            if tuple(t.shape) != tuple(new[k].shape):
                raise RuntimeError(f"re-pack changed the shape of {k}")
            t.copy_(new[k])
        from . import ops
        ops.refresh_thin_out(old.values())
        if hasattr(self, "_cond_cache"):
            self._cond_cache = None

    def fuse_lora(self, lora_state_dict: Mapping, lora_scale: float = 1.0, base_state_dict: Optional[Mapping] = None):
        base = base_state_dict if base_state_dict is not None else self._base_view()
        view = LoraFusedView(base, lora_state_dict, lora_scale)
        if not view.pairs:
            return self
        self._repack_in_place(view)
        self._lora = {"scale": float(lora_scale), "modules": len(view.pairs)}
        return self

    def unfuse_lora(self, base_state_dict: Optional[Mapping] = None):
        self._repack_in_place(base_state_dict if base_state_dict is not None else self._base_view())
        self._lora = None
        return self

    def load_lora_adapter(self, pretrained_model_name_or_path_or_dict, lora_scale: float = 1.0, **kw):
        sd = pretrained_model_name_or_path_or_dict
        if not isinstance(sd, Mapping):
            sd = LazyCheckpoint([Path(sd)])
        return self.fuse_lora(sd, lora_scale, **kw)


def save_reference_checkpoint(state_dict: Mapping, config: Mapping, directory, variant: Optional[str] = None) -> Path:
    from safetensors.torch import save_file
    d = Path(directory)
    d.mkdir(parents=True, exist_ok=True)
    cfg = {k: (list(v) if isinstance(v, tuple) else v) for k, v in dict(config).items()}
    (d / CONFIG_NAME).write_text(json.dumps(cfg, indent=2, default=str))
    stem = WEIGHTS_NAME + (f".{variant}" if variant else "")
    save_file({k: v.detach().contiguous().cpu() for k, v in state_dict.items()}, str(d / f"{stem}.safetensors"))
    return d
```

### diffusers_amd/ops.py

```python
from __future__ import annotations

import ctypes as C
import os
import threading
import weakref
from typing import Optional

import torch

from . import _lib as L
from . import tuning

bf16 = torch.bfloat16

DEFAULT_STAGING = L.STAGE_LDS_DIRECT
DEFAULT_TILE = L.TILE_AUTO
TUNING = True

PREFETCH = os.environ.get("DIFFUSERS_AMD_PREFETCH", "1") != "0"
_prefetch_tls = threading.local()


class WeightPrefetch:
    def __init__(self, models=(), owner=None, slots=()):
# ... 193 lines not shown
    if t.dtype not in dtypes or not t.is_cuda:
        kinds = " / ".join(str(d).replace("torch.", "").replace("bfloat16", "bf16").replace("float32", "fp32") for d in dtypes)
        raise ValueError(f"{name} must be a {kinds} HIP tensor (there is no CPU / fp32 fallback)")


def _rows2d(t: torch.Tensor, name: str) -> int:
    if t.dim() != 2 or t.stride(1) != 1:
        raise ValueError(f"{name}: expected a 2-D tensor with contiguous last dim, got shape {tuple(t.shape)} "
                         f"strides {t.stride()}")
    return t.stride(0) if t.shape[0] > 1 else max(t.stride(0), t.shape[1])


QKV_CANDIDATES = ((L.TILE_K2_128x80, L.STAGE_PINGPONG), (L.TILE_K2_128x80, L.STAGE_PINGPONG3), (L.TILE_K2_128x160, L.STAGE_PINGPONG),
                  (L.TILE_K2_128x160, L.STAGE_LDS_DIRECT), (L.TILE_K1_128x256, L.STAGE_LDS_DIRECT), (L.TILE_K1_128x256, L.STAGE_LDS_DIRECT3),
                  (L.TILE_K1_256x128, L.STAGE_LDS_DIRECT), (L.TILE_K1_256x128, L.STAGE_LDS_DIRECT3))
QKV_RETUNE = os.environ.get("DIFFUSERS_AMD_QKV_RETUNE", "0") == "1"
_qkv_retuned = set()
QKV_TILE_COLS = {L.TILE_K2_128x80: 80, L.TILE_K2_128x160: 160, L.TILE_K1_128x256: 256, L.TILE_K1_256x128: 128}


def qkv_variant(p: "L.GemmParams", stream: int):
    key = "qkv:" + tuning.key_of(p)
    ent = tuning.table().get(key) if TUNING else None
    if ent is not None and not (QKV_RETUNE and key not in _qkv_retuned):
        return ent[0], ent[1]
    _qkv_retuned.add(key)
    field = QKV_CANDIDATES if tuning.FAMILY == "all" else tuple(c for c in QKV_CANDIDATES if c[0] < L.TILE_K1_128x320)
    ok = [(t, s) for t, s in field if p.vt_col0 % QKV_TILE_COLS[t] == 0]
    if not ok:
        raise ValueError(f"linear(vt_out=): column origin {p.vt_col0} is not a multiple of a tile width {sorted(set(QKV_TILE_COLS.values()))}")
    if not (TUNING and tuning.LIVE) or torch.cuda.is_current_stream_capturing():
        return ok[0]
    lib, best = L.load(), None
    for t, s in ok:
        p.tile, p.staging, p.split_k = t, s, 1
        if lib.da_gemm_bf16(C.byref(p), stream) != 0:
            continue
        e0, e1 = torch.cuda.Event(enable_timing=True), torch.cuda.Event(enable_timing=True)
        e0.record()
        for _ in range(3):
            lib.da_gemm_bf16(C.byref(p), stream)
        e1.record()
        e1.synchronize()
        us = e0.elapsed_time(e1) * 1e3 / 3
        if best is None or us < best[2]:
            best = (t, s, us)
    if best is None:
        raise RuntimeError("linear(vt_out=): no kernel variant accepted this problem")
    tuning.table()[key] = (best[0], best[1], best[2], 1)
    tuning.mark_dirty()
    return best[0], best[1]


XATTN = os.environ.get("DIFFUSERS_AMD_XATTN", "0") == "1"
KV_PREFETCH = os.environ.get("DIFFUSERS_AMD_KV_PREFETCH", "0") == "1"
XATTN_MAX_KEYS = 80
XATTN_STAGING = L.STAGE_PINGPONG if os.environ.get("DIFFUSERS_AMD_XATTN_STAGE", "pp") == "pp" else L.STAGE_LDS_DIRECT
XATTN_MIN_TILES = int(os.environ.get("DIFFUSERS_AMD_XATTN_MIN_TILES", "0"))


def xattn_eligible(M: int, N: int, seq: int, head_dim: int, skv_alloc: int) -> bool:
    return head_dim == 64 and N % 128 == 0 and seq > 0 and seq % 128 == 0 and M % seq == 0 and M > 8 and \
        0 < skv_alloc <= XATTN_MAX_KEYS and skv_alloc % 8 == 0


def linear_qkv(x: torch.Tensor, wqkv: torch.Tensor, col0: int, bias: Optional[torch.Tensor] = None, ln: Optional[tuple] = None):
    M = x.shape[0]
    vt = torch.empty((wqkv.shape[0] - col0, M), device=x.device, dtype=bf16)
    qk = linear(x, wqkv, bias, ln=ln, vt_out=(vt, col0))
    return qk, vt


def linear(x: torch.Tensor, w: torch.Tensor, bias: Optional[torch.Tensor] = None, *, act: int = L.ACT_NONE,
           residual: Optional[torch.Tensor] = None, rowvec: Optional[torch.Tensor] = None, rows_per_batch: int = 0,
           alpha: float = 1.0, out_scale: float = 1.0, out: Optional[torch.Tensor] = None, out_f32: bool = False,
           bias_rows: Optional[torch.Tensor] = None, gate: Optional[torch.Tensor] = None,
           tile: Optional[int] = None, staging: Optional[int] = None, split_k: Optional[int] = None,
           stats_out: Optional[RowStats] = None, ln: Optional[tuple] = None, k_valid: int = 0,
           prefetch: Optional[torch.Tensor] = None, vt_out: Optional[tuple] = None,
           xattn: Optional[dict] = None) -> torch.Tensor:
    p, st = _linear_params(x, w, bias, act=act, residual=residual, rowvec=rowvec, rows_per_batch=rows_per_batch,
                           alpha=alpha, out_scale=out_scale, out=out, out_f32=out_f32, bias_rows=bias_rows, gate=gate,
                           tile=tile, staging=staging, split_k=split_k, stats_out=stats_out, ln=ln, k_valid=k_valid,
                           prefetch=prefetch, vt_out=vt_out, xattn=xattn)
    if p is None:
        return st
    _launch_gemm(p, st, "da_gemm_bf16(linear)")
    return p._out


def linear_pair(a: dict, b: dict):
    if a["x"].shape[0] <= 8 or b["x"].shape[0] <= 8:
        return linear(**a), linear(**b)
    pa, st = _linear_params(**a)
    pb, _ = _linear_params(**b)
    if pa is None or pb is None:
        raise ValueError("linear_pair: both problems must take the MFMA GEMM path (M > 8)")
    lib = L.load()
    pair = tuning.lookup_pair(pa, pb, st) if TUNING else None
    if pair is not None:
        sep = (tuning.table().get(tuning.key_of(pa)), tuning.table().get(tuning.key_of(pb)))
        if all(sep) and pair[2] >= sep[0][2] + sep[1][2]:
            pair = None
    if pair is None:
        _launch_gemm(pa, st, "da_gemm_bf16(linear)")
        _launch_gemm(pb, st, "da_gemm_bf16(linear)")
    else:
        pa.tile, pa.staging, pa.split_k, pb.split_k = pair[0], pair[1], 1, 1
        L.check(lib.da_gemm_pair_bf16(C.byref(pa), C.byref(pb), st), "da_gemm_pair_bf16")
    return pa._out, pb._out


def _linear_params(x: torch.Tensor, w: torch.Tensor, bias: Optional[torch.Tensor] = None, *, act: int = L.ACT_NONE,
                   residual: Optional[torch.Tensor] = None, rowvec: Optional[torch.Tensor] = None,
                   rows_per_batch: int = 0, alpha: float = 1.0, out_scale: float = 1.0,
                   out: Optional[torch.Tensor] = None, out_f32: bool = False, bias_rows: Optional[torch.Tensor] = None,
                   gate: Optional[torch.Tensor] = None, tile: Optional[int] = None, staging: Optional[int] = None,
                   split_k: Optional[int] = None, stats_out: Optional[RowStats] = None, ln: Optional[tuple] = None,
                   k_valid: int = 0, prefetch: Optional[torch.Tensor] = None, vt_out: Optional[tuple] = None,
                   xattn: Optional[dict] = None):
    _req(x, "x"), _req(w, "w")
    M, K = x.shape
    N, Kw = w.shape
    if K != Kw:
        raise ValueError(f"linear: K mismatch {K} vs {Kw}")
    n_out = N // 2 if act in (L.ACT_GEGLU, L.ACT_GEGLU_TANH) else N
    if vt_out is not None:
        vt_t, vt_col0 = vt_out
        _req(vt_t, "vt_out")
        if vt_t.dim() != 2 or vt_t.stride(1) != 1 or vt_t.shape[0] != N - vt_col0 or vt_t.shape[1] < M or not 0 < vt_col0 < N:
            raise ValueError("linear(vt_out=): expected (bf16 [N - col0][>= M], col0)")
        if M <= 8 or act != L.ACT_NONE or residual is not None or gate is not None or rowvec is not None or stats_out is not None:
            raise ValueError("linear(vt_out=): plain / LayerNorm-folded projections of more than 8 rows only")
        n_out = vt_col0
    if M <= 8 and act in (L.ACT_NONE, L.ACT_SILU, L.ACT_GELU_TANH) and rowvec is None and not out_f32 \
            and alpha == 1.0 and out_scale == 1.0 and bias_rows is None and gate is None and stats_out is None and ln is None:
        return None, linear_small_m(x, w, bias, act_out=act, residual=residual, out=out)
    if out is None:
        out = torch.empty((M, n_out), device=x.device, dtype=torch.float32 if out_f32 else bf16)
    p = L.GemmParams()
    p.A, p.A2, p.W, p.C = x.data_ptr(), None, w.data_ptr(), out.data_ptr()
    p.bias, p.rowvec, p.residual = _ptr(bias), _ptr(rowvec), _ptr(residual)
    p.M, p.N, p.K = M, N, K
    p.lda, p.ldw, p.ldc = _rows2d(x, "x"), _rows2d(w, "w"), _rows2d(out, "out")
    p.ldr = _rows2d(residual, "residual") if residual is not None else 0
    p.ld_rowvec = _rows2d(rowvec, "rowvec") if rowvec is not None else 0
    p.bias_rows, p.gate = _ptr(bias_rows), _ptr(gate)
    p.ld_gate = _rows2d(gate, "gate") if gate is not None else 0
    _prefetch_hook(p, x, w)
    if prefetch is not None:
        p.prefetch, p.prefetch_bytes = prefetch.data_ptr(), (prefetch.numel() * prefetch.element_size()) & ~15
    if gate is not None:
        if gate.dtype not in (bf16, torch.float32):
            raise TypeError("linear: gate must be bf16 (Flux rounding) or float32 (Wan rounding)")
        p.gate_f32 = int(gate.dtype == torch.float32)
    inplace = residual is not None and out.data_ptr() == residual.data_ptr()
    if inplace and p.ldr != p.ldc:
        raise ValueError("linear: an aliased residual must have the output's row stride")
    p.rows_per_batch = rows_per_batch
    p.alpha, p.out_scale, p.act, p.out_f32, p.conv = alpha, out_scale, act, int(out_f32), 0
    if not 0 <= k_valid <= K:
        raise ValueError(f"linear: k_valid {k_valid} outside [0, K = {K}]")
    p.k_valid = 0 if k_valid == K else k_valid
    st = _stream()
    if ln is not None:
        rs, fold = ln
        if rs.parts <= 0 or rs.buf.shape[0] != M or fold.s.numel() != N or fold.c.numel() != N:
            raise ValueError("linear(ln=): statistics / fold vectors do not match this problem (was the producer run?)")
        p.ln_stats, p.ln_stats_ld, p.ln_parts = rs.buf.data_ptr(), rs.buf.shape[1] * 2, rs.parts
        p.ln_s, p.ln_c, p.ln_eps = fold.s.data_ptr(), fold.c.data_ptr(), fold.eps
    if vt_out is not None:
        p.vt, p.vt_col0, p.ld_vt = vt_out[0].data_ptr(), int(vt_out[1]), vt_out[0].stride(0)
    if xattn is not None:
        xk, xvt = xattn["k"], xattn["vt"]
        _req(xk, "xattn k"), _req(xvt, "xattn vt")
        if not xattn_eligible(M, N, xattn["seq"], 64, xattn["skv_alloc"]) or xk.shape[1] != N or xvt.shape[0] != N:
            raise ValueError("linear(xattn=): heads of 64 channels in pairs (N % 128 == 0), row tiles of 128 inside one batch, "
                             f"<= {XATTN_MAX_KEYS} text tokens")
        if act != L.ACT_NONE or residual is not None or gate is not None or rowvec is not None or stats_out is not None \
                or vt_out is not None or out_f32 or out_scale != 1.0 or bias_rows is not None or M <= 8:
            raise ValueError("linear(xattn=): nothing but bias / the LayerNorm fold combines with the attention epilogue")
        p.xa_k, p.xa_vt = xk.data_ptr(), xvt.data_ptr()
        p.xa_skv, p.xa_skv_alloc, p.xa_k_ld, p.xa_vt_ld = int(xattn["skv"]), int(xattn["skv_alloc"]), _rows2d(xk, "xattn k"), _rows2d(xvt, "xattn vt")
        p.xa_scale = float(xattn["scale"])
        p.rows_per_batch = int(xattn["seq"])
        p._keep_xa = (xk, xvt)
        if tile is None:
            tile, staging, split_k = L.TILE_K2_128x128, XATTN_STAGING, 1
    tile_given = tile is not None
    if vt_out is not None and tile is None:
        tile, staging = qkv_variant(p, st)
        split_k = 1
    if (stats_out is not None or ln is not None) and tile is None:
        geglu_ = act in (L.ACT_GEGLU, L.ACT_GEGLU_TANH)
        ent = tuning.table().get(tuning.key_of(p)) if TUNING else None
        k3_geglu = (geglu_ and LN_FOLD_K3 and ent is not None and ent[0] == L.TILE_K3_256x320 and ln is not None and stats_out is None
                    and M % 256 == 0 and N % 320 == 0)
        if geglu_ and not k3_geglu and ent is not None and ent[0] in (L.TILE_K1_256x256, L.TILE_K1_128x256, L.TILE_K1_256x128,
                                                                      L.TILE_K1_256x320, L.TILE_K3_256x256, L.TILE_K3_256x320):
            ent = (L.TILE_K1_128x320, L.STAGE_LDS_DIRECT) + tuple(ent[2:])
        k2_ok = (ent is not None and ent[0] in ((L.TILE_K1_128x320, L.TILE_K3_256x320) if geglu_ else (L.TILE_K2_128x80, L.TILE_K2_128x160))
                 and not out_f32 and p.ldc % 8 == 0 and out.data_ptr() % 16 == 0 and N % 16 == 0 and gate is None
                 and (residual is None or (p.ldr % 8 == 0 and residual.data_ptr() % 16 == 0))
                 and not (ent[0] == L.TILE_K2_128x160 and ent[1] in (L.STAGE_LDS_DIRECT3, L.STAGE_PINGPONG3))
                 and not (geglu_ and ent[1] != L.STAGE_LDS_DIRECT))
        if k2_ok and LN_FOLD_K2:
            tile, staging, split_k = ent[0], ent[1], 1
        else:
            tile, staging, split_k = ((L.TILE_128x128, L.STAGE_LDS_DIRECT) if geglu_ else (L.TILE_128x64, L.STAGE_LDS_DIRECT3)) + (1,)
    _select_variant(p, tile, staging, st, inplace=inplace, split_k=split_k, device=x.device)
    if stats_out is not None:
        if act in (L.ACT_GEGLU, L.ACT_GEGLU_TANH) or out_f32 or stats_out.buf.shape[0] != M:
            raise ValueError("linear(stats_out=): bf16 non-GEGLU outputs only, one statistics row per output row")
        p.stats_out, p.stats_ld = stats_out.buf.data_ptr(), stats_out.buf.shape[1] * 2
        stats_out.parts = int(L.load().da_gemm_stats_parts(C.byref(p)))
        if stats_out.parts > STATS_MAX_CONSUMED and not tile_given:
            p.tile, p.staging, p.split_k = (L.TILE_128x128 if N <= 128 * STATS_MAX_CONSUMED else L.TILE_128x256), L.STAGE_LDS_DIRECT, 1
            stats_out.parts = int(L.load().da_gemm_stats_parts(C.byref(p)))
        if not 0 < stats_out.parts <= min(stats_out.buf.shape[1], STATS_MAX_CONSUMED):
            raise ValueError(f"linear(stats_out=): {stats_out.parts} column tiles: the consumer reads at most "
                             f"{STATS_MAX_CONSUMED} partials per row (use a wider tile for this producer)")
    p._out = out
    p._keep = (x, w, bias, residual, rowvec, bias_rows, gate, stats_out, ln, vt_out)
    return p, st


def conv2d_nhwc(x: torch.Tensor, w: torch.Tensor, bias: Optional[torch.Tensor] = None, *, ksize: int = 3,
                x2: Optional[torch.Tensor] = None, stride: int = 1, up: bool = False, pad: Optional[int] = None,
                rowvec: Optional[torch.Tensor] = None, residual: Optional[torch.Tensor] = None,
                out_scale: float = 1.0, act: int = L.ACT_NONE, tile: Optional[int] = None,
                staging: Optional[int] = None, pad_after: int = 0, out: Optional[torch.Tensor] = None,
                split_k: Optional[int] = None, k_valid: int = 0) -> torch.Tensor:
    _req(x, "x"), _req(w, "w")
    if x2 is not None:
        _req(x2, "x2")
    p = _conv_params(x, w, ksize, x2, stride, up, pad, pad_after)
    B, Hout, Wout, Cout = x.shape[0], p.Hout, p.Wout, p.N
    if out is None:
        out = torch.empty((B, Hout, Wout, Cout), device=x.device, dtype=bf16)
    else:
        _req(out, "out")
        if tuple(out.shape) != (B, Hout, Wout, Cout) or not out.is_contiguous():
            raise ValueError("conv2d_nhwc: out must be contiguous [B][Hout][Wout][Cout]")
    inplace = residual is not None and residual.data_ptr() == out.data_ptr()
    p.A, p.A2, p.W, p.C = x.data_ptr(), _ptr(x2), w.data_ptr(), out.data_ptr()
    p.bias, p.rowvec, p.residual = _ptr(bias), _ptr(rowvec), _ptr(residual)
    if residual is not None:
        _req(residual, "residual")
        if tuple(residual.shape) != (B, Hout, Wout, Cout) or not residual.is_contiguous():
            raise ValueError("conv2d_nhwc: residual must be contiguous [B][Hout][Wout][Cout]")
        p.ldr = Cout
    if rowvec is not None:
        _req(rowvec, "rowvec")
        p.ld_rowvec = _rows2d(rowvec, "rowvec")
        p.rows_per_batch = Hout * Wout
    p.alpha, p.out_scale, p.act, p.out_f32 = 1.0, out_scale, act, 0
    C1, C2 = p.C1, p.C2
    if not 0 <= k_valid <= C1 or (k_valid and C2):
        raise ValueError(f"conv2d_nhwc: k_valid {k_valid} outside [0, C1 = {C1}] (or given with a second source)")
    p.k_valid = 0 if k_valid == C1 else k_valid
    _prefetch_hook(p, x, w)
    st = _stream()
    _select_variant(p, tile, staging, st, inplace=inplace, split_k=split_k, device=x.device)
    _launch_gemm(p, st, "da_gemm_bf16(conv)")
    return out


def _conv_params(x: torch.Tensor, w: torch.Tensor, ksize: int, x2: Optional[torch.Tensor], stride: int, up: bool,
                 pad: Optional[int], pad_after: int) -> "L.GemmParams":
    B, H, W_, C1 = x.shape
    C2 = 0
    if x2 is not None:
        if x2.shape[:3] != x.shape[:3]:
            raise ValueError("conv2d_nhwc: x2 spatial shape mismatch")
        C2 = x2.shape[3]
    if not x.is_contiguous() or (x2 is not None and not x2.is_contiguous()):
        raise ValueError("conv2d_nhwc: inputs must be contiguous NHWC")
    Cout, K = w.shape
    if K != ksize * ksize * (C1 + C2):
        raise ValueError(f"conv2d_nhwc: weight K={K} != {ksize}*{ksize}*{C1 + C2}")
    if pad is None:
        pad = (ksize - 1) // 2
    Hv, Wv = (2 * H, 2 * W_) if up else (H, W_)
    Hout = (Hv + 2 * pad + pad_after - ksize) // stride + 1
    Wout = (Wv + 2 * pad + pad_after - ksize) // stride + 1
    p = L.GemmParams()
    p.M, p.N, p.K = B * Hout * Wout, Cout, K
    p.lda, p.ldw, p.ldc = 0, K, Cout
    p.conv = ksize
    p.Hin, p.Win, p.C1, p.C2, p.Hout, p.Wout = H, W_, C1, C2, Hout, Wout
    p.stride, p.up, p.pad = stride, int(up), pad
    return p


def conv_chunk_channels(x: torch.Tensor, w: torch.Tensor, tile: int, *, ksize: int = 3, x2: Optional[torch.Tensor] = None,
                        stride: int = 1, up: bool = False, pad: Optional[int] = None, pad_after: int = 0) -> int:
    p = _conv_params(x, w, ksize, x2, stride, up, pad, pad_after)
    r = int(L.load().da_conv_chunk_channels(C.byref(p), int(tile)))
    if r < 0:
        L.check(-r, f"da_conv_chunk_channels(tile {L.TILE_NAMES[tile] if 0 <= tile < len(L.TILE_NAMES) else tile})")
    return r


def linear_small_m(x: torch.Tensor, w: torch.Tensor, bias: Optional[torch.Tensor] = None, *, act_in: int = L.ACT_NONE,
                   act_out: int = L.ACT_NONE, residual: Optional[torch.Tensor] = None,
                   out: Optional[torch.Tensor] = None) -> torch.Tensor:
    _req(x, "x"), _req(w, "w")
    M, K = x.shape
    N = w.shape[0]
    if w.shape[1] != K or not w.is_contiguous():
        raise ValueError("linear_small_m: weight must be contiguous [N][K]")
    if out is None:
        out = torch.empty((M, N), device=x.device, dtype=bf16)
    L.check(L.load().da_linear_small_m_bf16(
        x.data_ptr(), w.data_ptr(), _ptr(bias), _ptr(residual), out.data_ptr(), M, N, K, _rows2d(x, "x"),
        _rows2d(out, "out"), _rows2d(residual, "residual") if residual is not None else 0, act_in, act_out, _stream()),
        "da_linear_small_m_bf16")
    return out


def pack_geglu(w: torch.Tensor, bias: Optional[torch.Tensor]):
    n2 = w.shape[0]
    n = n2 // 2
    if n % 64:
        raise ValueError("pack_geglu: inner dim must be a multiple of 64")
    idx = torch.arange(n, device=w.device).view(n // 32, 32)
    order = torch.cat([idx, idx + n], dim=1).reshape(-1)
    wp = w.index_select(0, order).contiguous()
    bp = bias.index_select(0, order).contiguous() if bias is not None else None
    return wp, bp


def pack_conv_weight(w: torch.Tensor) -> torch.Tensor:
    co, ci, kh, kw = w.shape
    return w.permute(0, 2, 3, 1).reshape(co, kh * kw * ci).contiguous()


def attention(q: torch.Tensor, k: torch.Tensor, vt: torch.Tensor, *, B: int, H: int, D: int, Sq: int, Skv: int,
              Skv_alloc: int, q_row_stride: int, k_row_stride: int, q_batch_stride: int, k_batch_stride: int,
              vt_ld: int, vt_batch_stride: int, scale: Optional[float] = None,
              out: Optional[torch.Tensor] = None, ring_slots: int = 0, causal: bool = False,
              bias: Optional[torch.Tensor] = None, q_block: int = 0, pv_delay: int = 0, algo: int = 0,
              kv_split: int = 0) -> torch.Tensor:
    _req(q, "q"), _req(k, "k"), _req(vt, "vt")
    if out is None:
        out = torch.empty((B * Sq, H * D), device=q.device, dtype=bf16)
    o_row_stride = _rows2d(out, "out")
    p = L.AttentionParams()
    p.q, p.k, p.vt, p.out = q.data_ptr(), k.data_ptr(), vt.data_ptr(), out.data_ptr()
    p.B, p.H, p.Sq, p.Skv, p.Skv_alloc, p.D = B, H, Sq, Skv, Skv_alloc, D
    p.q_batch_stride, p.k_batch_stride, p.vt_batch_stride = q_batch_stride, k_batch_stride, vt_batch_stride
    p.o_batch_stride = Sq * o_row_stride
    p.q_row_stride, p.k_row_stride, p.vt_ld, p.o_row_stride = q_row_stride, k_row_stride, vt_ld, o_row_stride
    p.scale = (D ** -0.5) if scale is None else scale
    p.ring_slots = ring_slots
    p.q_block = q_block
    p.pv_delay = pv_delay
    p.algo = algo
    p.causal = int(causal)
    p.kv_split = kv_split if ATTN_SPLIT or kv_split > 1 else 1
    if p.kv_split != 1 and bias is None and not causal and D in (64, 128) and Skv >= 256 and B * H * ((Sq + 127) // 128) >= 64:
        ws = attn_split_workspace(q.device, _stream())
        p.split_ws, p.split_ws_bytes = ws.data_ptr(), ws.numel()
    if bias is not None:
        _req(bias, "bias", None)
        if bias.dtype not in (bf16, torch.float32) or bias.dim() != 4 or bias.stride(3) != 1 or \
                (bias.shape[2] != 1 and bias.shape[2] < Sq):
            raise ValueError("attention: bias must be a bf16 / fp32 [B|1][H|1][Sq|1][>= ceil64(Skv)] tensor, last dim contiguous")
        if bias.shape[0] not in (1, B) or bias.shape[1] not in (1, H):
            raise ValueError("attention: bias batch / head dims must be 1 or match")
        p.bias, p.bias_f32 = bias.data_ptr(), int(bias.dtype == torch.float32)
        p.bias_batch_stride = bias.stride(0) if bias.shape[0] > 1 else 0
        p.bias_head_stride = bias.stride(1) if bias.shape[1] > 1 else 0
        p.bias_row_stride = bias.stride(2) if bias.shape[2] > 1 else 0
    L.check(L.load().da_attention_bf16(C.byref(p), _stream()), "da_attention_bf16")
    return out


def softmax_rows(scores: torch.Tensor, out: Optional[torch.Tensor] = None) -> torch.Tensor:
    _req(scores, "scores", torch.float32)
    M, N = scores.shape
    if out is None:
        out = torch.empty((M, (N + 3) // 4 * 4), device=scores.device, dtype=bf16)[:, :N]
    else:
        _req(out, "out")
        if out.shape[0] != M or out.shape[1] < N:
            raise ValueError("softmax_rows: out must be [M][>= N]")
    if _rows2d(scores, "scores") % 4 or _rows2d(out, "out") % 4:
        raise ValueError("softmax_rows: the row strides of scores and out must be multiples of 4 (view a wider buffer)")
    L.check(L.load().da_softmax_rows_f32_bf16(scores.data_ptr(), out.data_ptr(), M, N, _rows2d(scores, "scores"),
                                              _rows2d(out, "out"), _stream()), "da_softmax_rows_f32_bf16")
    return out


_gn_ws = {}
GN_MULTI = os.environ.get("DIFFUSERS_AMD_GN_MULTI", "0") == "1"
_gn_sync = {}


def gn_sync_workspace(device: torch.device, stream: int) -> torch.Tensor:
    key = (device.index if device.index is not None else torch.cuda.current_device(), stream)
    ws = _gn_sync.get(key)
    if ws is None:
        ws = torch.zeros(int(L.load().da_groupnorm_sync_bytes()), dtype=torch.uint8, device=device)
        _gn_sync[key] = ws
    return ws


def gn_sync_error(device=None) -> bool:
    off = 4096 * 4
    return any(bool(w[off:off + 4].view(torch.int32).item()) for (d, _), w in _gn_sync.items()
               if device is None or d == torch.device(device).index)


def group_norm_nhwc(x: torch.Tensor, gamma: torch.Tensor, beta: torch.Tensor, groups: int, eps: float,
                    silu: bool = False, x2: Optional[torch.Tensor] = None) -> torch.Tensor:
    _req(x, "x"), _req(gamma, "gamma"), _req(beta, "beta")
    if not x.is_contiguous() or (x2 is not None and not x2.is_contiguous()):
        raise ValueError("group_norm_nhwc: contiguous channels-last input required")
    B = x.shape[0]
    C1 = x.shape[-1]
    Ctot = C1 + (x2.shape[-1] if x2 is not None else 0)
    HW = x.numel() // (B * C1)
    lib = L.load()
    nbytes = lib.da_groupnorm_workspace_bytes(B, HW, Ctot, groups)
    ws = torch.empty((max(nbytes, 4) // 4,), device=x.device, dtype=torch.float32)
    y = torch.empty(tuple(x.shape[:-1]) + (Ctot,), device=x.device, dtype=bf16)
    sync = gn_sync_workspace(x.device, _stream()).data_ptr() if GN_MULTI and B * HW * Ctot >= (1 << 20) else None
    L.check(lib.da_groupnorm_nhwc_bf16(x.data_ptr(), _ptr(x2), C1, gamma.data_ptr(), beta.data_ptr(), y.data_ptr(),
                                       ws.data_ptr(), B, HW, Ctot, groups, eps, L.ACT_SILU if silu else L.ACT_NONE,
                                       sync, _stream()), "da_groupnorm_nhwc_bf16")
    return y


def rms_norm(x: torch.Tensor, gamma: torch.Tensor, eps: float) -> torch.Tensor:
    _req(x, "x"), _req(gamma, "gamma")
    M, Cc = x.shape
    y = torch.empty((M, Cc), device=x.device, dtype=bf16)
    L.check(L.load().da_rmsnorm_bf16(x.data_ptr(), gamma.data_ptr(), y.data_ptr(), M, Cc, _rows2d(x, "x"), Cc, eps, _stream()),
            "da_rmsnorm_bf16")
    return y


def rmsnorm_channels(x: torch.Tensor, gamma: torch.Tensor, *, real_channels: int, silu: bool = False) -> torch.Tensor:
    _req(x, "x"), _req(gamma, "gamma")
    Cc = x.shape[-1]
    if not x.is_contiguous() or gamma.numel() != Cc:
        raise ValueError("rmsnorm_channels: contiguous channels-last input and a [C] gamma required")
    y = torch.empty_like(x)
    L.check(L.load().da_rmsnorm_channels_bf16(x.data_ptr(), gamma.data_ptr(), y.data_ptr(), x.numel() // Cc, Cc,
                                              float(real_channels) ** 0.5, L.ACT_SILU if silu else L.ACT_NONE,
                                              _stream()), "da_rmsnorm_channels_bf16")
    return y


def layer_norm(x: torch.Tensor, gamma: Optional[torch.Tensor], beta: Optional[torch.Tensor], eps: float, *,
               mod_scale: Optional[torch.Tensor] = None, mod_shift: Optional[torch.Tensor] = None,
               rows_per_batch: int = 0) -> torch.Tensor:
    _req(x, "x")
    M, Cc = x.shape
    y = torch.empty((M, Cc), device=x.device, dtype=bf16)
    mod_ld = _rows2d(mod_scale, "mod_scale") if mod_scale is not None else 0
    mod_f32 = 0
    if mod_scale is not None:
        if mod_scale.dtype != mod_shift.dtype or mod_scale.dtype not in (bf16, torch.float32):
            raise TypeError("layer_norm: mod_scale / mod_shift must both be bf16 or both float32")
        mod_f32 = int(mod_scale.dtype == torch.float32)
    L.check(L.load().da_layernorm_bf16(x.data_ptr(), _ptr(gamma), _ptr(beta), y.data_ptr(), _ptr(mod_scale),
                                       _ptr(mod_shift), mod_ld, mod_f32, rows_per_batch, M, Cc, _rows2d(x, "x"), Cc,
                                       eps, _stream()), "da_layernorm_bf16")
    return y


def rmsnorm_rope_(x: torch.Tensor, *, heads: int, head_dim: int, col_offsets, weights=None, eps: float = 1e-6,
                  cos: Optional[torch.Tensor] = None, sin: Optional[torch.Tensor] = None, rope_row0: int = 0,
                  rows_per_batch: int = 0, norm: str = "per_head") -> torch.Tensor:
    _req(x, "x")
    rows = x.shape[0]
    ld = _rows2d(x, "x")
    parts = len(col_offsets)
    offs = (C.c_int * parts)(*[int(o) for o in col_offsets])
    wptr = None
    if weights is not None:
        for w_ in weights:
            if w_ is not None:
                _req(w_, "weight")
        wptr = (C.c_void_p * parts)(*[(w_.data_ptr() if w_ is not None else None) for w_ in weights])
    if cos is not None:
        _req(cos, "cos", torch.float32), _req(sin, "sin", torch.float32)
        if cos.shape[-1] != head_dim or not cos.is_contiguous() or not sin.is_contiguous():
            raise ValueError("rmsnorm_rope_: cos / sin must be contiguous [rows][head_dim] fp32")
    mode = {"none": 0, "per_head": 1, "across_heads": 2}[norm]
    L.check(L.load().da_rmsnorm_rope_bf16(x.data_ptr(), ld, rows, rows_per_batch or rows, heads, head_dim, parts, offs,
                                          wptr, eps, _ptr(cos), _ptr(sin), rope_row0, mode, _stream()),
            "da_rmsnorm_rope_bf16")
    return x


def _dt(t: torch.Tensor) -> int:
    if t.dtype == bf16:
        return L.DTYPE_BF16
    if t.dtype == torch.float32:
        return L.DTYPE_F32
    raise TypeError(f"sampler kernels support bf16 / fp32 latents, got {t.dtype}")


def _check_sampler(what: str, x: torch.Tensor, model_out: torch.Tensor, out: Optional[torch.Tensor], cfg: bool,
                   same_dtype: bool = True) -> None:
    _req(x, "sample", None), _req(model_out, "model_output", None)
    if model_out.numel() != x.numel() * (2 if cfg else 1):
        raise ValueError(f"{what}: model_output must hold {'[2 x sample] (uncond, cond)' if cfg else 'as many'} "
                         f"elements{'' if cfg else ' as the sample'} (got {model_out.numel()} vs {x.numel()})")
    if same_dtype and model_out.dtype != x.dtype:
        raise TypeError(f"{what}: model_output ({model_out.dtype}) and sample ({x.dtype}) must have the same dtype")
    if not x.is_contiguous() or not model_out.is_contiguous():
        raise ValueError(f"{what}: sample and model_output must be contiguous")
    if out is not None:
        _req(out, "out", None)
        if out.numel() != x.numel() or not out.is_contiguous():
            raise ValueError(f"{what}: out must be a contiguous tensor of the sample's size")


def euler_scale_model_input(x: torch.Tensor, table: torch.Tensor, step_idx: torch.Tensor, rep: int = 1) -> torch.Tensor:
    _req(x, "x", None)
    if not x.is_contiguous():
        raise ValueError("euler_scale_model_input: contiguous sample required")
    out = torch.empty((rep * x.shape[0],) + tuple(x.shape[1:]), device=x.device, dtype=x.dtype)
    L.check(L.load().da_euler_scale_model_input(x.data_ptr(), out.data_ptr(), table.data_ptr(), step_idx.data_ptr(),
                                                rep, x.numel(), _dt(x), _stream()), "da_euler_scale_model_input")
    return out


def euler_step(eps: torch.Tensor, x: torch.Tensor, table: torch.Tensor, step_idx: torch.Tensor, *, cfg: bool,
               guidance: float, out: Optional[torch.Tensor] = None, pred_type: int = L.PRED_EPSILON) -> torch.Tensor:
    _check_sampler("euler_step", x, eps, out, cfg)
    if out is None:
        out = torch.empty_like(x)
    elif out.dtype != x.dtype:
        raise TypeError("euler_step: out must have the sample's dtype")
    L.check(L.load().da_euler_step(eps.data_ptr(), x.data_ptr(), out.data_ptr(), table.data_ptr(), step_idx.data_ptr(),
                                   int(cfg), guidance, x.numel(), _dt(x), int(pred_type), _stream()), "da_euler_step")
    return out


def euler_ancestral_step(eps: torch.Tensor, x: torch.Tensor, noise: torch.Tensor, table: torch.Tensor, step_idx: torch.Tensor, *,
                         cfg: bool, guidance: float, out: Optional[torch.Tensor] = None, pred_type: int = L.PRED_EPSILON,
                         noise_step_stride: int = 0) -> torch.Tensor:
    for t_, name in ((eps, "model_output"), (x, "sample"), (noise, "noise"), (table, "table"), (step_idx, "step_idx")):
        if not torch.is_tensor(t_) or not t_.is_cuda:
            raise ValueError(f"euler_ancestral_step: {name} must be a HIP device tensor (there is no CPU path)")
    if out is not None and not out.is_cuda:
        raise ValueError("euler_ancestral_step: out must be a HIP device tensor (there is no CPU path)")
    if x.dtype not in (bf16, torch.float32):
        raise ValueError(f"euler_ancestral_step: bf16 / fp32 samples, got {x.dtype}")
    if eps.dtype != x.dtype:
        raise ValueError(f"euler_ancestral_step: model_output ({eps.dtype}) and sample ({x.dtype}) must have the same dtype")
    if pred_type not in (L.PRED_EPSILON, L.PRED_V):
        raise ValueError("euler_ancestral_step: pred_type must be epsilon or v_prediction")
    _check_sampler("euler_ancestral_step", x, eps, out, cfg)
    if out is None:
        out = torch.empty_like(x)
    elif out.dtype != x.dtype:
        raise ValueError("euler_ancestral_step: out must have the sample's dtype")
    if table.dtype != torch.float32 or table.dim() != 2 or table.shape[1] != 8 or not table.is_contiguous():
        raise ValueError("euler_ancestral_step: table must be a contiguous [steps][8] fp32 tensor")
    if step_idx.dtype != torch.int32:
        raise ValueError("euler_ancestral_step: step_idx must be an int32 device scalar")
    if noise.dtype != eps.dtype:
        raise ValueError(f"euler_ancestral_step: noise ({noise.dtype}) must have the model output's dtype ({eps.dtype})")
    stride = int(noise_step_stride)
    if stride < 0 or not noise.is_contiguous():
        raise ValueError("euler_ancestral_step: noise must be contiguous, with a step stride >= 0")
    if noise.numel() < (table.shape[0] - 1) * stride + x.numel():
        raise ValueError(f"euler_ancestral_step: noise holds {noise.numel()} elements, {table.shape[0]} rows of stride {stride} "
                         f"and a sample of {x.numel()} need {(table.shape[0] - 1) * stride + x.numel()}")
    L.check(L.load().da_euler_ancestral_step(eps.data_ptr(), x.data_ptr(), noise.data_ptr(), stride, out.data_ptr(),
                                             table.data_ptr(), step_idx.data_ptr(), int(cfg), float(guidance), x.numel(), _dt(x),
                                             int(pred_type), _stream()), "da_euler_ancestral_step")
    return out


def x0_linear_step(eps: torch.Tensor, x: torch.Tensor, noise: Optional[torch.Tensor], table: torch.Tensor,
                   step_idx: torch.Tensor, *, cfg: bool, guidance: float,
                   out: Optional[torch.Tensor] = None, noise_step_stride: int = 0,
                   pred_type: int = L.PRED_EPSILON) -> torch.Tensor:
    _check_sampler("x0_linear_step", x, eps, out, cfg)
    if out is None:
        out = torch.empty_like(x)
    elif out.dtype != x.dtype:
        raise TypeError("x0_linear_step: out must have the sample's dtype")
    if noise is not None:
        _req(noise, "noise", None)
        if noise.dtype != x.dtype or not noise.is_contiguous():
            raise ValueError("x0_linear_step: noise must be contiguous and have the dtype of the sample")
        if noise.numel() < x.numel() or (noise_step_stride and noise.numel() % x.numel()):
            raise ValueError("x0_linear_step: noise must hold one sample-sized block (per step, with a step stride)")
    L.check(L.load().da_x0_linear_step(eps.data_ptr(), x.data_ptr(), _ptr(noise), noise_step_stride, out.data_ptr(),
                                       table.data_ptr(),
                                       step_idx.data_ptr(), int(cfg), guidance, x.numel(), _dt(x), int(pred_type),
                                       _stream()),
            "da_x0_linear_step")
    return out


def flowmatch_step(v: torch.Tensor, x: torch.Tensor, table: torch.Tensor, step_idx: torch.Tensor, *, cfg: bool = False,
                   guidance: float = 0.0, out: Optional[torch.Tensor] = None) -> torch.Tensor:
# ... 397 lines not shown
```

Baseline: 1.031 images/s.

## Replace nearest-2x upsample conv3x3 with sub-pixel 2x2 collapsed-weight implicit GEMM

Nearest-2x upsampling followed by a 3x3 conv is rewritten as four parity-specific 2x2 convs over the low-resolution input, using weights collapsed ahead of time. This cuts the reduction from 9*Cin to 4*Cin per output pixel and reads the un-upsampled input directly. A new SUBPX mode of the implicit-GEMM kernel maps each output tile to one of the four parities and scatters results to interleaved output rows. Costs are extra weight storage, a scattered store pattern, and bf16 rounding of the summed weights, which can change results slightly.

```diff
diff --git a/diffusers_amd/csrc/gemm.hip b/diffusers_amd/csrc/gemm.hip
--- a/diffusers_amd/csrc/gemm.hip
+++ b/diffusers_amd/csrc/gemm.hip
@@ -7,6 +7,7 @@
 namespace da_gemm2 {
 int dispatch_lin(const da_gemm_params& p, int tile, int staging, hipStream_t s);
 int dispatch_conv(const da_gemm_params& p, int tile, int staging, hipStream_t s);
+int dispatch_conv_subpx(const da_gemm_params& p, int tile, int staging, hipStream_t s);
 }
 namespace da_gemm3 {
 int dispatch_lin(const da_gemm_params& p, int tile, int staging, hipStream_t s);
@@ -42,12 +43,14 @@
 
 int validate_conv(const da_gemm_params& p) {
   if (p.C1 <= 0 || (p.C1 & 63) || (p.C2 & 63) || p.C2 < 0) return DA_ERR_UNSUPPORTED;
-  if (p.conv != 1 && p.conv != 3) return DA_ERR_UNSUPPORTED;
+  const bool subpx = da_gemm2::is_subpixel(p);
+  if (p.conv != 1 && p.conv != 3 && !subpx) return DA_ERR_UNSUPPORTED;
   if (p.K != p.conv * p.conv * (p.C1 + p.C2)) return DA_ERR_INVALID;
   if (p.stride != 1 && p.stride != 2) return DA_ERR_UNSUPPORTED;
-  if (p.up != 0 && p.up != 1) return DA_ERR_INVALID;
+  if (p.up != 0 && p.up != 1 && !subpx) return DA_ERR_INVALID;
   if (p.Hin <= 0 || p.Win <= 0 || p.Hout <= 0 || p.Wout <= 0) return DA_ERR_INVALID;
   if (p.M % (p.Hout * p.Wout)) return DA_ERR_INVALID;
+  if (subpx && (p.C2 != 0 || p.stride != 1 || p.Hout != 2 * p.Hin || p.Wout != 2 * p.Win || p.ldw != p.K)) return DA_ERR_INVALID;
   return DA_OK;
 }
 
@@ -64,6 +67,9 @@
     const int v = validate_conv(p);
     if (v != DA_OK) return v;
     if (p.C2 > 0 && !p.A2) return DA_ERR_INVALID;
+    if (da_gemm2::is_subpixel(p) && (p.residual || p.rowvec || p.gate || p.bias_rows || p.out_f32 || p.act != DA_ACT_NONE ||
+                                     p.split_k > 1 || p.stats_out || p.ln_stats || p.vt || p.xa_k || p.k_valid))
+      return DA_ERR_UNSUPPORTED;
   } else {
     if ((p.lda & 7) || (p.ldw & 7)) return DA_ERR_UNSUPPORTED;
   }
@@ -92,6 +98,7 @@
 
 bool tile_ok(const da_gemm_params& p, int tile) {
   if (tile <= 0 || tile >= kNumTiles) return false;
+  if (da_gemm2::is_subpixel(p) && !is_k2(tile)) return false;
   if (is_k3(tile)) {
     if (p.conv || p.split_k > 1 || p.stats_out || (p.ln_stats && tile != DA_TILE_K3_256x320) || p.vt || p.xa_k) return false;
     if (tile == DA_TILE_K3_256x320)
@@ -136,6 +143,7 @@
   if (is_k3(tile)) return pb ? DA_ERR_UNSUPPORTED : da_gemm3::dispatch_lin(p, tile, staging, s);
   if (is_k2(tile)) {
     if (pb) return DA_ERR_UNSUPPORTED;
+    if (da_gemm2::is_subpixel(p)) return da_gemm2::dispatch_conv_subpx(p, tile, staging, s);
     return p.conv ? da_gemm2::dispatch_conv(p, tile, staging, s) : da_gemm2::dispatch_lin(p, tile, staging, s);
   }
   if (p.conv) return pb ? DA_ERR_UNSUPPORTED : da_gemm::dispatch_conv(p, tile, staging, s);
diff --git a/diffusers_amd/csrc/gemm2_kernel.cuh b/diffusers_amd/csrc/gemm2_kernel.cuh
--- a/diffusers_amd/csrc/gemm2_kernel.cuh
+++ b/diffusers_amd/csrc/gemm2_kernel.cuh
@@ -19,7 +19,7 @@
 
 
 template <int KG, int WM, int WN, int MT, int NT, int NSLOT, bool CONV, bool PP = false, bool STREAMW = false, bool GIL = false,
-          bool LNF = false, int XA = 0>
+          bool LNF = false, int XA = 0, bool SUBPX = false>
 __global__ __launch_bounds__(512) void igemm2_bf16_kernel(const da_gemm_params p, const int xcd_gx_chunk) {
 #if defined(__HIP_DEVICE_COMPILE__)
   const int xcd_gx = xcd_gx_chunk & 255;
@@ -28,6 +28,7 @@
   constexpr int PX = BM / 8, PW = BN / 8;
   constexpr int XBYTES = BM * 128, SLICE = (BM + BN) * 128, PAIR = KG * SLICE;
   static_assert(!PP || KG == 2, "ping-pong is a property of the two K-groups");
+  static_assert(!SUBPX || (CONV && !LNF && XA == 0), "sub-pixel nearest-2x conv: a mode of the implicit-GEMM conv");
   static_assert(!STREAMW || (KG == 1 && NSLOT == 2 && !CONV), "streaming-W loop: one K-group, two-slice ring, nn.Linear");
   static_assert(!GIL || (KG == 1 && !CONV && WN == 2 && (NT % 2) == 0), "GEGLU-interleaved ownership: two wave columns, value / gate tile pairs");
   static_assert(!LNF || (!CONV && !STREAMW), "LayerNorm fold: nn.Linear instantiations of the ring loops");
@@ -59,7 +60,9 @@
   const int wm = wq / WN, wn = wq - wm * WN;
   const int r16 = lane & 15, kq = lane >> 4;
 
-  const int tiles_n = (p.N + BN - 1) / BN, tiles_m = (p.M + BM - 1) / BM;
+  const int Mr = SUBPX ? (p.M >> 2) : p.M;
+  const int tiles_par = SUBPX ? (Mr + BM - 1) / BM : 0;
+  const int tiles_n = (p.N + BN - 1) / BN, tiles_m = SUBPX ? 4 * tiles_par : (p.M + BM - 1) / BM;
   const int gyn = 8 / xcd_gx;
   const int tm_per = (tiles_m + gyn - 1) / gyn, tn_per = (tiles_n + xcd_gx - 1) / xcd_gx;
   const int bid = (int)blockIdx.x;
@@ -68,7 +71,8 @@
   const int lm = kblk / tn_per, ln = kblk - lm * tn_per;
   const int tm = gy * tm_per + lm, tn = gx * tn_per + ln;
   if (tm >= tiles_m || tn >= tiles_n) return;
-  const int m0 = tm * BM, n0 = tn * BN;
+  const int par = SUBPX ? tm / tiles_par : 0, py = par >> 1, px = par & 1;
+  const int m0 = (SUBPX ? tm - par * tiles_par : tm) * BM, n0 = tn * BN;
 
   const uint16_t* __restrict__ A = (const uint16_t*)p.A;
   const uint16_t* __restrict__ A2 = (const uint16_t*)p.A2;
@@ -76,7 +80,8 @@
   const int nk = p.K >> 6;
   const int nk2 = (nk + KG - 1) / KG;
   const int Ctot = CONV ? (p.C1 + p.C2) : 0;
-  const int Hv = CONV ? (p.Hin << p.up) : 0, Wv = CONV ? (p.Win << p.up) : 0;
+  const int ups = SUBPX ? 0 : p.up;
+  const int Hv = CONV ? (p.Hin << ups) : 0, Wv = CONV ? (p.Win << ups) : 0;
 
   int x_h[XI], x_r[XI], w_h[WI], w_r[WI];
   bool x_ok[XI], w_ok[WI];
@@ -100,7 +105,25 @@
   constexpr int my_loads = XI + WI;
 
   int xr_base[XI], xr_oy[XI], xr_ox[XI];
-  if constexpr (CONV) {
+  if constexpr (SUBPX) {
+    const int hw = p.Hin * p.Win;
+#pragma unroll
+    for (int i = 0; i < XI; ++i) {
+      const int m = m0 + x_r[i] * 8 + (lane >> 3);
+      if (m < Mr) {
+        const int b = m / hw;
+        const int rem = m - b * hw;
+        const int y = rem / p.Win;
+        xr_base[i] = b * p.Hin;
+        xr_oy[i] = y + py - 1;
+        xr_ox[i] = (rem - y * p.Win) + px - 1;
+      } else {
+        xr_base[i] = 0;
+        xr_oy[i] = -100000;
+        xr_ox[i] = -100000;
+      }
+    }
+  } else if constexpr (CONV) {
     const int hw = p.Hout * p.Wout;
 #pragma unroll
     for (int i = 0; i < XI; ++i) {
@@ -122,7 +145,14 @@
 
   size_t xbase = 0, xbytes = 0x7fffffff, x2bytes = 0x7fffffff;
   int pb = 0;
-  if constexpr (CONV) {
+  if constexpr (SUBPX) {
+    const int hw = p.Hin * p.Win;
+    const int b0 = m0 / hw;
+    const int y0 = (m0 - b0 * hw) / p.Win;
+    pb = __builtin_amdgcn_readfirstlane((b0 * p.Hin + max(0, y0 + py - 1)) * p.Win);
+    const size_t pix_left = (size_t)Mr - (size_t)pb;
+    xbytes = min(pix_left * p.C1 * 2, (size_t)0x7fffffff);
+  } else if constexpr (CONV) {
     const int hw = p.Hout * p.Wout;
     const int b0 = m0 / hw;
     const int oy0 = (m0 - b0 * hw) / p.Wout;
@@ -135,7 +165,7 @@
   }
   __amdgpu_buffer_rsrc_t rs_x = uniform_rsrc(A + (CONV ? (size_t)pb * p.C1 : xbase), xbytes);
   __amdgpu_buffer_rsrc_t rs_x2 = uniform_rsrc((CONV && A2) ? A2 + (size_t)pb * p.C2 : A, x2bytes);
-  __amdgpu_buffer_rsrc_t rs_w = uniform_rsrc(Wt + (size_t)n0 * p.ldw, 0x7fffffff);
+  __amdgpu_buffer_rsrc_t rs_w = uniform_rsrc(Wt + (SUBPX ? (size_t)par * p.N * p.ldw : 0) + (size_t)n0 * p.ldw, 0x7fffffff);
 
   int vo_x[XI], vo_x2[XI], vo_w[WI];
 #pragma unroll
@@ -166,7 +196,7 @@
       const int sc = (lane & 7) ^ ((row >> 1) & 7);
       const int iy = xr_oy[i] + c_kh[h], ix = xr_ox[i] + c_kw[h];
       const bool ok = (unsigned)iy < (unsigned)Hv && (unsigned)ix < (unsigned)Wv;
-      const int rel = (xr_base[i] + (iy >> p.up)) * p.Win + (ix >> p.up) - pb;
+      const int rel = (xr_base[i] + (iy >> ups)) * p.Win + (ix >> ups) - pb;
       vo_x[i] = ok ? (rel * p.C1 + sc * 8) * 2 : (int)0x80000000;
       vo_x2[i] = ok ? (rel * p.C2 + sc * 8) * 2 : (int)0x80000000;
     }
@@ -261,6 +291,17 @@
   static_assert(SPLIT_M || (NT % 2) == 0, "one of the wave tile's dimensions must split between the two K-groups");
   constexpr int MH = (KG == 2 && SPLIT_M) ? MT / 2 : MT, NH = (KG == 1 || SPLIT_M) ? NT : NT / 2;
   const bool geglu = (p.act == DA_ACT_GEGLU || p.act == DA_ACT_GEGLU_TANH);
+  auto out_row = [&](int m) {
+    if constexpr (SUBPX) {
+      const int hw = p.Hin * p.Win;
+      const int b = m / hw;
+      const int rem = m - b * hw;
+      const int y = rem / p.Win;
+      return ((b * p.Hin + y) * 2 + py) * p.Wout + 2 * (rem - y * p.Win) + px;
+    } else {
+      return m;
+    }
+  };
   auto row_of = [&](int ih) { return m0 + (wm * MT + (SPLIT_M ? g * MH : 0) + ih) * 16 + r16; };
   auto col_tile = [&](int jh) { return GIL ? 4 * (jh >> 1) + 2 * (jh & 1) + wn : wn * NT + (SPLIT_M ? 0 : g * NH) + jh; };
   auto col_of = [&](int jh) { return n0 + col_tile(jh) * 16 + 4 * kq; };
@@ -905,7 +946,7 @@
           if (NPIECE % 64 != 0 && q >= NPIECE) continue;
           const int row = q / PPR, c8 = q % PPR;
           const int mo = band_row0(ih) + row, no = band_col0 + c8 * 8;
-          const bool inside = mo < p.M && no < p.N;
+          const bool inside = mo < Mr && no < p.N;
           uint4 pk;
           if constexpr (PACKED) {
             pk = *(const uint4*)(stg + row * (ROWB / 2) + c8 * 16);
@@ -921,7 +962,7 @@
             for (int e = 0; e < 8; ++e) o[e] *= p.out_scale;
             pk.x = pack_bf2(o[0], o[1]); pk.y = pack_bf2(o[2], o[3]); pk.z = pack_bf2(o[4], o[5]); pk.w = pack_bf2(o[6], o[7]);
           }
-          if (inside) *(uint4*)((uint16_t*)p.C + (size_t)mo * p.ldc + no) = pk;
+          if (inside) *(uint4*)((uint16_t*)p.C + (size_t)out_row(mo) * p.ldc + no) = pk;
           if constexpr (LNF) {
             if (p.stats_out) {
               float r[8];
@@ -959,7 +1000,7 @@
 #pragma unroll
     for (int ih = 0; ih < MH; ++ih) {
       const int m = row_of(ih);
-      if (m >= p.M) continue;
+      if (m >= Mr) continue;
       const int bidx = (GATE != 0 || (!PF && has_rowvec)) ? (m / p.rows_per_batch) : 0;
       const float brow = bias_rows ? bf2f(bias_rows[m]) : 0.f;
 #pragma unroll
@@ -977,12 +1018,12 @@
         else if (has_res) rsv = *(const uint2*)((const uint16_t*)p.residual + (size_t)m * p.ldr + n);
         epilogue4<ACT, GATE, true>(p, o, n, bidx, brow, bias_v[jh], rvv, rsv);
         if (p.out_f32) {
-          *(float4*)((float*)p.C + (size_t)m * p.ldc + n) = make_float4(o[0], o[1], o[2], o[3]);
+          *(float4*)((float*)p.C + (size_t)out_row(m) * p.ldc + n) = make_float4(o[0], o[1], o[2], o[3]);
         } else {
           uint2 pk;
           pk.x = pack_bf2(o[0], o[1]);
           pk.y = pack_bf2(o[2], o[3]);
-          *(uint2*)((uint16_t*)p.C + (size_t)m * p.ldc + n) = pk;
+          *(uint2*)((uint16_t*)p.C + (size_t)out_row(m) * p.ldc + n) = pk;
         }
       }
     }
@@ -1051,12 +1092,12 @@
 
 
 template <int KG, int WM, int WN, int MT, int NT, int NSLOT, bool CONV, bool PP = false, bool STREAMW = false, bool GIL = false,
-          bool LNF = false, int XA = 0>
+          bool LNF = false, int XA = 0, bool SUBPX = false>
 int launch(const da_gemm_params& p, hipStream_t s) {
   constexpr int BM = 16 * MT * WM, BN = 16 * NT * WN;
   const LaunchGeom geom = launch_geom(p, BM, BN, CONV);
   constexpr size_t lds = (size_t)NSLOT * KG * (BM + BN) * 128 + 1024 + (LNF ? 2 * BN * 4 : 0);
-  auto kern = igemm2_bf16_kernel<KG, WM, WN, MT, NT, NSLOT, CONV, PP, STREAMW, GIL, LNF, XA>;
+  auto kern = igemm2_bf16_kernel<KG, WM, WN, MT, NT, NSLOT, CONV, PP, STREAMW, GIL, LNF, XA, SUBPX>;
   static bool attr_set = false;
   if (!attr_set) {
     if (hipFuncSetAttribute((const void*)kern, hipFuncAttributeMaxDynamicSharedMemorySize, (int)lds) != hipSuccess)
@@ -1068,6 +1109,7 @@
   return DA_OK;
 }
 
+#if !defined(DA_GEMM2_SUBPX_ONLY)
 inline int stats_band_cols(int tile) { return (tile == DA_TILE_K2_128x80 || tile == DA_TILE_K2_128x160) ? 80 : 0; }
 
 inline int dispatch_lnf(const da_gemm_params& p, int tile, int staging, hipStream_t s) {
@@ -1126,6 +1168,58 @@
   return DA_ERR_UNSUPPORTED;
 }
 
+#else
+
+inline int dispatch_subpx(const da_gemm_params& p, int tile, int staging, hipStream_t s) {
+  if (p.split_k > 1 || !staging_fits(p) || p.stats_out || p.ln_stats || p.vt || p.xa_k) return DA_ERR_UNSUPPORTED;
+  const int ns = (staging == DA_STAGE_LDS_DIRECT || staging == DA_STAGE_PINGPONG) ? 2
+                 : (staging == DA_STAGE_LDS_DIRECT3 || staging == DA_STAGE_PINGPONG3) ? 3 : 0;
+  if (ns == 0) return DA_ERR_UNSUPPORTED;
+#define DA2_SUBPX(KG, WM, WN, MT, NT, NS, PP) launch<KG, WM, WN, MT, NT, NS, true, PP, false, false, false, 0, true>(p, s)
+  if (staging == DA_STAGE_PINGPONG || staging == DA_STAGE_PINGPONG3) {
+    switch (tile) {
+      case DA_TILE_K2_128x128:
+        if (ns == 2) return DA2_SUBPX(2, 2, 2, 4, 4, 2, true);
+        break;
+      case DA_TILE_K2_128x80:
+        return ns == 2 ? DA2_SUBPX(2, 4, 1, 2, 5, 2, true) : DA2_SUBPX(2, 4, 1, 2, 5, 3, true);
+      case DA_TILE_K2_128x160:
+        if (ns == 2) return DA2_SUBPX(2, 2, 2, 4, 5, 2, true);
+        break;
+      case DA_TILE_K2_128x64:
+        return ns == 2 ? DA2_SUBPX(2, 2, 2, 4, 2, 2, true) : DA2_SUBPX(2, 2, 2, 4, 2, 3, true);
+    }
+    return DA_ERR_UNSUPPORTED;
+  }
+  switch (tile) {
+    case DA_TILE_K2_128x128:
+      if (ns == 2) return DA2_SUBPX(2, 2, 2, 4, 4, 2, false);
+      break;
+    case DA_TILE_K2_128x80:
+      return ns == 2 ? DA2_SUBPX(2, 4, 1, 2, 5, 2, false) : DA2_SUBPX(2, 4, 1, 2, 5, 3, false);
+    case DA_TILE_K2_128x160:
+      if (ns == 2) return DA2_SUBPX(2, 2, 2, 4, 5, 2, false);
+      break;
+    case DA_TILE_K2_128x64:
+      return ns == 2 ? DA2_SUBPX(2, 2, 2, 4, 2, 2, false) : DA2_SUBPX(2, 2, 2, 4, 2, 3, false);
+    case DA_TILE_K1_128x320:
+      if (ns == 2) return DA2_SUBPX(1, 4, 2, 2, 10, 2, false);
+      break;
+    case DA_TILE_K1_256x128:
+      return ns == 2 ? DA2_SUBPX(1, 4, 2, 4, 4, 2, false) : DA2_SUBPX(1, 4, 2, 4, 4, 3, false);
+    case DA_TILE_K1_128x256:
+      return ns == 2 ? DA2_SUBPX(1, 2, 4, 4, 4, 2, false) : DA2_SUBPX(1, 2, 4, 4, 4, 3, false);
+    case DA_TILE_K1_256x160:
+      if (ns == 2) return DA2_SUBPX(1, 4, 2, 4, 5, 2, false);
+      break;
+  }
+#undef DA2_SUBPX
+  return DA_ERR_UNSUPPORTED;
+}
+
+#endif
+
+#if !defined(DA_GEMM2_SUBPX_ONLY)
 template <bool CONV>
 int dispatch(const da_gemm_params& p, int tile, int staging, hipStream_t s) {
   if (p.split_k > 1 || !staging_fits(p)) return DA_ERR_UNSUPPORTED;
@@ -1203,5 +1297,6 @@
   }
   return DA_ERR_UNSUPPORTED;
 }
+#endif
 
 }
diff --git a/diffusers_amd/csrc/gemm2_shared.cuh b/diffusers_amd/csrc/gemm2_shared.cuh
--- a/diffusers_amd/csrc/gemm2_shared.cuh
+++ b/diffusers_amd/csrc/gemm2_shared.cuh
@@ -105,12 +105,14 @@
   return (on && p.conv > 1) ? p.conv * p.conv : 1;
 }
 
+inline bool is_subpixel(const da_gemm_params& p) { return p.conv == 2 && p.up == 2; }
+
 struct LaunchGeom {
   int gx, grid;
   long long rows_xcd;
 };
 inline LaunchGeom launch_geom(const da_gemm_params& p, int BM, int BN, bool conv) {
-  const int tiles_m = (p.M + BM - 1) / BM, tiles_n = (p.N + BN - 1) / BN;
+  const int tiles_m = is_subpixel(p) ? 4 * ((p.M / 4 + BM - 1) / BM) : (p.M + BM - 1) / BM, tiles_n = (p.N + BN - 1) / BN;
   const int gx = choose_xcd_gx2(tiles_m, tiles_n, BM, BN, conv ? xcd_conv_weighting(p) : 1, conv ? (long long)(p.C1 + p.C2) * 2 : 0), gy = 8 / gx;
   const int tm_per = (tiles_m + gy - 1) / gy, tn_per = (tiles_n + gx - 1) / gx;
   const long long rows_xcd = (long long)BM * (tm_per < (32 + tn_per - 1) / tn_per ? tm_per : (32 + tn_per - 1) / tn_per);
diff --git a/diffusers_amd/csrc/gemm2_upconv.hip b/diffusers_amd/csrc/gemm2_upconv.hip
--- /dev/null
+++ b/diffusers_amd/csrc/gemm2_upconv.hip
@@ -0,0 +1,6 @@
+#define DA_GEMM2_SUBPX_ONLY
+#include "gemm2_kernel.cuh"
+
+namespace da_gemm2 {
+int dispatch_conv_subpx(const da_gemm_params& p, int tile, int staging, hipStream_t s) { return dispatch_subpx(p, tile, staging, s); }
+}
diff --git a/diffusers_amd/layers.py b/diffusers_amd/layers.py
--- a/diffusers_amd/layers.py
+++ b/diffusers_amd/layers.py
@@ -186,8 +186,15 @@
 
     def __init__(self, w: Weights, prefix: str):
         self.conv = Conv3x3(w, prefix + ".conv")
+        self.w_sub = None
+        if ops.UPCONV_SUBPIXEL:
+            wt = w.get(prefix + ".conv.weight")
+            if wt.shape[1] % 64 == 0:
+                self.w_sub = ops.collapse_upconv_weight(wt)
 
     def __call__(self, x):
+        if self.w_sub is not None and ops.UPCONV_SUBPIXEL and x.is_cuda:
+            return ops.conv2d_up2x_subpixel(x, self.w_sub, self.conv.bias)
         return self.conv(x, up=True)
 
 
diff --git a/diffusers_amd/loading.py b/diffusers_amd/loading.py
--- a/diffusers_amd/loading.py
+++ b/diffusers_amd/loading.py
@@ -185,6 +185,11 @@
     return h.hexdigest()[:24]
 
 
+def packed_inventory_tag() -> str:
+    from . import ops
+    return (f"+lnfold{int(ops.LN_FOLD)}qkv" if ops.LN_FOLD else "") + "+tembcat" + ("+upsubpx" if ops.UPCONV_SUBPIXEL else "")
+
+
 def read_config(d: Path) -> dict:
     cfg = json.loads((d / CONFIG_NAME).read_text())
     return {k: (tuple(v) if isinstance(v, list) else v) for k, v in cfg.items() if not k.startswith("_")}
@@ -207,9 +212,7 @@
         files = _weight_files(d, variant)
         cfg = read_config(d)
         cfg.update(config_overrides)
-        from . import ops
-        fp = checkpoint_fingerprint(files, extra=cls.__name__ + json.dumps(cfg, sort_keys=True, default=str)
-                                    + (f"+lnfold{int(ops.LN_FOLD)}qkv" if ops.LN_FOLD else "") + "+tembcat")
+        fp =checkpoint_fingerprint(files, extra=cls.__name__ + json.dumps(cfg, sort_keys=True, default=str) + packed_inventory_tag())
         cdir = Path(cache_dir) if cache_dir is not None else d / PACKED_DIR
         cfile = cdir / f"{cls.__name__}-{fp}.safetensors"
         model = None
diff --git a/diffusers_amd/ops.py b/diffusers_amd/ops.py
--- a/diffusers_amd/ops.py
+++ b/diffusers_amd/ops.py
@@ -519,6 +519,89 @@
     return r
 
 
+UPCONV_SUBPIXEL = os.environ.get("DIFFUSERS_AMD_UPCONV_SUBPIXEL", "1") != "0"
+UPCONV_TILES = (L.TILE_K2_128x128, L.TILE_K2_128x80, L.TILE_K2_128x160, L.TILE_K2_128x64, L.TILE_K1_128x320, L.TILE_K1_256x128,
+                L.TILE_K1_128x256, L.TILE_K1_256x160)
+
+
+def collapse_upconv_weight(w: torch.Tensor) -> torch.Tensor:
+    if w.dim() != 4 or tuple(w.shape[2:]) != (3, 3):
+        raise ValueError(f"collapse_upconv_weight: expected [Cout][Cin][3][3], got {tuple(w.shape)}")
+    co, ci = w.shape[:2]
+    a = w.float() if w.dtype in (torch.bfloat16, torch.float16) else w
+    rows = (torch.stack((a[:, :, 0], a[:, :, 1] + a[:, :, 2]), dim=2), torch.stack((a[:, :, 0] + a[:, :, 1], a[:, :, 2]), dim=2))
+    blocks = []
+    for py in (0, 1):
+        r = rows[py]
+        for px in (0, 1):
+            c = torch.stack((r[..., 0], r[..., 1] + r[..., 2]) if px == 0 else (r[..., 0] + r[..., 1], r[..., 2]), dim=3)
+            blocks.append(c.permute(0, 2, 3, 1).reshape(co, 4 * ci))
+    return torch.cat(blocks, dim=0).to(w.dtype).contiguous()
+
+
+def _upconv_params(x: torch.Tensor, w_sub: torch.Tensor) -> "L.GemmParams":
+    B, H, W_, C1 = x.shape
+    if not x.is_contiguous() or not w_sub.is_contiguous():
+        raise ValueError("conv2d_up2x_subpixel: x must be contiguous NHWC, w_sub contiguous")
+    if w_sub.dim() != 2 or w_sub.shape[1] != 4 * C1 or w_sub.shape[0] % 4:
+        raise ValueError(f"conv2d_up2x_subpixel: collapsed weight {tuple(w_sub.shape)} does not fit {C1} input channels "
+                         "(expected [4 * Cout][4 * Cin], ops.collapse_upconv_weight)")
+    p = L.GemmParams()
+    p.M, p.N, p.K = B * 4 * H * W_, w_sub.shape[0] // 4, 4 * C1
+    p.lda, p.ldw, p.ldc = 0, 4 * C1, p.N
+    p.conv, p.up, p.stride, p.pad = 2, 2, 1, 0
+    p.Hin, p.Win, p.C1, p.C2, p.Hout, p.Wout = H, W_, C1, 0, 2 * H, 2 * W_
+    return p
+
+
+def upconv_variant(p: "L.GemmParams"):
+    tab = tuning.table()
+    ent = tab.get(tuning.key_of(p))
+    if ent is None:
+        q = L.GemmParams()
+        q.M, q.N, q.K, q.conv, q.up, q.stride = p.M, p.N, 9 * p.C1, 3, 1, 1
+        q.Hin, q.Win, q.C1, q.C2 = p.Hin, p.Win, p.C1, 0
+        ent = tab.get(tuning.key_of(q))
+    if ent is not None and ent[0] in UPCONV_TILES and ent[3] <= 1:
+        return ent[0], ent[1]
+    return L.TILE_K2_128x128, L.STAGE_LDS_DIRECT
+
+
+def conv2d_up2x_subpixel(x: torch.Tensor, w_sub: torch.Tensor, bias: Optional[torch.Tensor] = None, *,
+                         tile: Optional[int] = None, staging: Optional[int] = None,
+                         out: Optional[torch.Tensor] = None) -> torch.Tensor:
+    _req(x, "x"), _req(w_sub, "w_sub")
+    p = _upconv_params(x, w_sub)
+    shape = (x.shape[0], p.Hout, p.Wout, p.N)
+    if out is None:
+        out = torch.empty(shape, device=x.device, dtype=bf16)
+    else:
+        _req(out, "out")
+        if tuple(out.shape) != shape or not out.is_contiguous():
+            raise ValueError("conv2d_up2x_subpixel: out must be contiguous [B][2H][2W][Cout]")
+    if bias is not None:
+        _req(bias, "bias")
+    p.A, p.W, p.C, p.bias = x.data_ptr(), w_sub.data_ptr(), out.data_ptr(), _ptr(bias)
+    p.alpha, p.out_scale, p.act, p.out_f32, p.split_k = 1.0, 1.0, L.ACT_NONE, 0, 1
+    _prefetch_hook(p, x, w_sub)
+    if tile is None and staging is None:
+        p.tile, p.staging = upconv_variant(p) if TUNING else (L.TILE_K2_128x128, L.STAGE_LDS_DIRECT)
+    else:
+        p.tile = L.TILE_K2_128x128 if tile is None else tile
+        p.staging = L.STAGE_LDS_DIRECT if staging is None else staging
+    p._auto = False
+    _launch_gemm(p, _stream(), "da_gemm_bf16(sub-pixel up-conv)")
+    return out
+
+
+def upconv_chunk_channels(x: torch.Tensor, w_sub: torch.Tensor, tile: int) -> int:
+    p = _upconv_params(x, w_sub)
+    r = int(L.load().da_conv_chunk_channels(C.byref(p), int(tile)))
+    if r < 0:
+        L.check(-r, "da_conv_chunk_channels(sub-pixel up-conv)")
+    return r
+
+
 def linear_small_m(x: torch.Tensor, w: torch.Tensor, bias: Optional[torch.Tensor] = None, *, act_in: int = L.ACT_NONE,
                    act_out: int = L.ACT_NONE, residual: Optional[torch.Tensor] = None,
                    out: Optional[torch.Tensor] = None) -> torch.Tensor:
```

Result: no change. 1.040 images/s, median of 6 (+0.9%).
